# shgaurav1/DVG

Measured on AMD Instinct MI355X. Metric: predicted frames/sec at 64x64, batch 64, 10-in/10-out, higher is better.
Workload: dtype f32; 1 GPU; Moving-MNIST 64x64 rollout (generate_frames.py make_gifs sample loop), vgg_64 + lstm + GP trigger sample at i%15==0, batch 64 per GPU, 10-in/10-out; model_family=vgg, batch_per_gpu=64, n_past=10, n_future=10, parallelism=replicas x1 (no data-path collective), launch=hipGraph replay, rollouts_in_flight=3, tile_policy=energy, loop_invariant_skip_halves=hoisted, upsample_conv3x3=as transposed 4x4/s2 conv, conv3x3_deep_layers=Winograd F(4x4,3x3) / F(2x2,3x3)

## Files before the change

dvg_amd/csrc/conv_igemm2.hip:

```cpp
#include <cstdlib>
#include <type_traits>

#include "dvg_common.h"

namespace dvg {

constexpr int DVG_GEMM_WGS_PER_CU = DVG_BF16X3 ? 3 : 4;
constexpr int DVG_GEMM128_WGS = DVG_BF16X3 ? 3 : 2;
constexpr int DVG_GEMM128_GT = DVG_BF16X3 ? 2 : 4;
constexpr int DVG_GEMM_GT = 4;
constexpr int DVG_GEMM128_MIN_WGS = 4 * 768;
[[maybe_unused]] constexpr int DVG_GEMM_NT2 = 256;
constexpr int DVG_TILE16_MIN_WGS = 256;

enum { M2_CONV3 = 0, M2_CONV4S2 = 1, M2_CONVT4S2 = 2, M2_GEMM = 3 };

struct Igemm2Params {
    const float* x;
    const float* skip;
    const float* w;
    const float* scale;
    const float* shift;
    float* y;
    float* y_pool;
// ... 1273 lines not shown
    const long total = (long)cout * cin * 12 / 2;
    const int nblk = cout >> 6;
    for (long i = blockIdx.x * (long)blockDim.x + threadIdx.x; i < total; i += (long)gridDim.x * blockDim.x) {
        const int k = (int)(i & 7) * 2;
        long r = i >> 3;
        const int co = r % cout; r /= cout;
        const int tap = r % 12;
        const int chunk = r / 12;
        const int row = tap >> 2, f = tap & 3;
        float u[2];
#pragma unroll
        for (int e = 0; e < 2; ++e) {
            const float* g = src + (((long)co * cin + chunk * 16 + k + e) * 3 + row) * 3;
            if (f == 0) u[e] = g[0];
            else if (f == 1) u[e] = ((g[0] + g[1]) + g[2]) * 0.5f;
            else if (f == 2) u[e] = ((g[0] - g[1]) + g[2]) * 0.5f;
            else u[e] = g[2];
        }
        wrow_store_pair(dst, (((size_t)chunk * nblk + (co >> 6)) * 12 + tap) * 64 + (co & 63), co & 63, k, u[0], u[1]);
    }
    wrow_drain();
}

__global__ void pack_k16_kernel(const float* __restrict__ src, float* __restrict__ dst, int cout, int cin, int kh,
                                int kw, int transposed) {
    const long total = (long)cout * cin * kh * kw / 2;
    const int nblk = cout >> 6, taps = kh * kw;
    for (long i = blockIdx.x * (long)blockDim.x + threadIdx.x; i < total; i += (long)gridDim.x * blockDim.x) {
        const int k = (int)(i & 7) * 2;
        long r = i >> 3;
        const int co = r % cout; r /= cout;
        const int t = r % taps;
        const int chunk = r / taps;
        const int ci = chunk * 16 + k, a = t / kw, b = t % kw;
        const long j = transposed ? ((((long)ci * cout + co) * kh + (kh - 1 - a)) * kw + (kw - 1 - b))
                                  : ((((long)co * cin + ci) * kh + a) * kw + b);
        const long j1 = j + (transposed ? (long)cout * kh * kw : (long)kh * kw);
        int slot = t;
        if (transposed && kh == 4 && kw == 4) {
            const int py = a & 1, px = b & 1;
            slot = (py * 2 + px) * 4 + ((2 + py - a) >> 1) * 2 + ((2 + px - b) >> 1);
        } else if (kh == 4 && kw == 4) {
            slot = ((a & 1) * 2 + (b & 1)) * 4 + (a >> 1) * 2 + (b >> 1);
        }
        wrow_store_pair(dst, (((size_t)chunk * nblk + (co >> 6)) * taps + slot) * 64 + (co & 63), co & 63, k, src[j], src[j1]);
    }
    wrow_drain();
}

}

using namespace dvg;

extern "C" int dvg_mfma_mode(void) { return DVG_BF16X3 ? 1 : 0; }
extern "C" int dvg_packed_row_floats(void) { return DVG_WROW; }

extern "C" void dvg_debug_set_clockbuf(void* buf, unsigned records) {
    g_clk = (unsigned long long*)buf;
    g_clk_cap = buf ? records : 0;
}

extern "C" int dvg_pack_conv_weight_k16(const float* w, float* w_packed, int cout, int cin, int kh, int kw,
                                        int transposed, void* stream) {
    DVG_REQUIRE(w && w_packed, DVG_ERR_NULL, "dvg_pack_conv_weight_k16: NULL pointer");
    DVG_REQUIRE(cout > 0 && cout % 64 == 0 && cin > 0 && cin % 16 == 0 && kh > 0 && kw > 0, DVG_ERR_SHAPE,
                "dvg_pack_conv_weight_k16: Cin must be a multiple of 16, Cout of 64");
    const long total = (long)cout * cin * kh * kw / 2;
    long g = (total + 255) / 256;
    if (g > 4096) g = 4096;
    hipLaunchKernelGGL(pack_k16_kernel, dim3((unsigned)g), dim3(256), 0, (hipStream_t)stream, w, w_packed, cout, cin, kh,
                       kw, transposed);
    return check_launch("dvg_pack_conv_weight_k16");
}

static long v2_wgs(int mode, int N, int Hg, int Wg, int Cout, int ti, int th, int tw) {
    return (long)((N + ti - 1) / ti) * (Hg / th) * (Wg / tw) * (Cout / 64) * (mode == M2_CONVT4S2 ? 4 : 1);
}

static int v2_splits(int mode, int N, int Hg, int Wg, int Cout, int Cin, int ti, int th, int tw) {
    if (tw == 16) return 1;
    return choose_splitk(v2_wgs(mode, N, Hg, Wg, Cout, ti, th, tw), Cin / 16);
}

extern "C" int dvg_conv_splitk_v2(int mode, int N, int H, int W, int Cin, int Cout) {
    int Hg = H, Wg = W;
    if (mode == M2_CONV4S2) { Hg = H / 2; Wg = W / 2; }
    int ti, th, tw;
    if (Cin % 16 || Cout % 64 || tile2(mode, N, Hg, Wg, Cout, &ti, &th, &tw)) return -1;
    return v2_splits(mode, N, Hg, Wg, Cout, Cin, ti, th, tw);
}

extern "C" int dvg_conv_stats_rows_v2(int mode, int N, int H, int W, int Cin, int Cout, int pool, int with_workspace) {
    int Hg = H, Wg = W;
    if (mode == M2_CONV4S2) { Hg = H / 2; Wg = W / 2; }
    int ti, th, tw;
    if (tile2(mode, N, Hg, Wg, Cout, &ti, &th, &tw)) return -1;
    if (with_workspace && v2_splits(mode, N, Hg, Wg, Cout, Cin, ti, th, tw) > 1) {
        int Ho = H, Wo = W;
        if (mode == M2_CONV4S2) { Ho = H / 2; Wo = W / 2; }
        if (mode == M2_CONVT4S2) { Ho = 2 * H; Wo = 2 * W; }
        const long units = pool ? (long)N * (Ho / 2) * (Wo / 2) : (long)N * Ho * Wo;
        const int upb = finish_units_per_block(units);
        return (int)((units + upb - 1) / upb);
    }
    return ((N + ti - 1) / ti) * (Hg / th) * (Wg / tw) * (mode == M2_CONVT4S2 ? 4 : 1);
}

static int checks2(const Igemm2Params& p, const char* who) {
    DVG_REQUIRE(p.x && p.w && p.y, DVG_ERR_NULL, "%s: x/w/y must not be NULL", who);
    DVG_REQUIRE((p.skip != nullptr) == (p.C2 > 0), DVG_ERR_SHAPE, "%s: skip pointer / C2 mismatch", who);
    DVG_REQUIRE(p.N > 0 && p.H > 0 && p.W > 0, DVG_ERR_SHAPE, "%s: empty shape", who);
    DVG_REQUIRE(p.C1 > 0 && p.C1 % 16 == 0 && p.C2 % 16 == 0, DVG_ERR_SHAPE, "%s: C1=%d C2=%d must be multiples of 16",
                who, p.C1, p.C2);
    DVG_REQUIRE(p.Cout > 0 && p.Cout % 64 == 0, DVG_ERR_SHAPE, "%s: Cout=%d must be a multiple of 64", who, p.Cout);
    DVG_REQUIRE(aligned16(p.x) && aligned16(p.w) && aligned16(p.y) && aligned16(p.skip), DVG_ERR_ALIGN,
                "%s: pointers must be 16-byte aligned", who);
    DVG_REQUIRE(p.act >= DVG_ACT_NONE && p.act <= DVG_ACT_SIGMOID, DVG_ERR_SHAPE, "%s: bad act", who);
    return DVG_OK;
}

#define D2(MODE, TI_, TH_, TW_) \
    if (ti == TI_ && th == TH_ && tw == TW_)                                             \
        return launch2<MODE, TI_, TH_, TW_>(p, Hg, Wg, workspace, workspace_floats, (hipStream_t)stream);



extern "C" int dvg_conv3x3_bn_act_v2(const float* x, const float* skip, const float* w_k16, const float* scale,
                                     const float* shift, float* y, float* y_pool, float* stats, int N, int H, int W,
                                     int C1, int C2, int Cout, int upsample_x, int act, float slope,
                                     float* workspace, long workspace_floats, const float* addend,
                                     const int* addend_map, int addend_block, void* stream) {
    Igemm2Params p{x, skip, w_k16, scale, shift, y, y_pool, stats, N, H, W, C1, C2, Cout, upsample_x ? 1 : 0, act, slope,
                   0, 0, 0, 0, 0, 1, 0, nullptr};
    p.addend = addend;
    p.add_map = addend ? addend_map : nullptr;
    p.add_B = addend_block;
    DVG_REQUIRE(p.add_map == nullptr || (addend_block > 0 && N % addend_block == 0), DVG_ERR_SHAPE,
                "dvg_conv3x3_bn_act_v2: addend_block must divide N");
    if (int e = checks2(p, "dvg_conv3x3_bn_act_v2")) return e;
    DVG_REQUIRE(aligned16(addend) && (addend == nullptr || y_pool == nullptr), DVG_ERR_SHAPE,
                "dvg_conv3x3_bn_act_v2: addend must be 16-byte aligned and excludes the pooled output");
    DVG_REQUIRE(H % 8 == 0 && W % 8 == 0, DVG_ERR_SHAPE, "dvg_conv3x3_bn_act_v2: H=%d W=%d must be multiples of 8", H, W);
    int Hg = H, Wg = W, ti, th, tw;
    DVG_REQUIRE(tile2(M2_CONV3, N, Hg, Wg, Cout, &ti, &th, &tw) == 0 && ti == 1, DVG_ERR_SHAPE,
                "dvg_conv3x3_bn_act_v2: no tile for %dx%d", H, W);
    D2(M2_CONV3, 1, 8, 16)
    D2(M2_CONV3, 1, 8, 8)
    return fail(DVG_ERR_SHAPE, "dvg_conv3x3_bn_act_v2: no kernel");
}

extern "C" int dvg_conv3x3_first_pair(const float* frame, const float* w0, const float* scale0, const float* shift0,
                                      const float* w1_k16, const float* scale1, const float* shift1, float* y, float* y_pool,
                                      int N, int H, int W, int Cout, int act, float slope, int y_from, void* stream) {
    DVG_REQUIRE(frame && w0 && scale0 && shift0, DVG_ERR_NULL, "dvg_conv3x3_first_pair: NULL pointer");
    DVG_REQUIRE(y_from >= 0 && y_from <= N && (y_from == 0 || y_pool != nullptr) && (y != nullptr || y_from == N), DVG_ERR_SHAPE,
                "dvg_conv3x3_first_pair: y_from=%d needs 0 <= y_from <= N, a pooled output when > 0, y unless == N", y_from);
    float* const y_biased = y ? y - (size_t)y_from * H * W * Cout : y_pool;
    Igemm2Params p{frame , nullptr, w1_k16, scale1, shift1, y_biased, y_pool, nullptr, N, H, W, 64, 0, Cout, 0,
                   act, slope, 0, 0, 0, 0, 0, 1, 0, nullptr};
    p.first_frame = frame; p.first_w = w0; p.first_scale = scale0; p.first_shift = shift0; p.first_slope = 0.2f;
    p.y_from = y_from;
    if (int e = checks2(p, "dvg_conv3x3_first_pair")) return e;
    DVG_REQUIRE(H % 8 == 0 && W % 16 == 0 && (long)N * (H / 8) * (W / 16) * (Cout / 64) >= 512, DVG_ERR_SHAPE,
                "dvg_conv3x3_first_pair: H %% 8, W %% 16 and >= 512 workgroups needed (N=%d H=%d W=%d Cout=%d)", N, H, W, Cout);
    return launch2<M2_CONV3, 1, 8, 16, 1, true>(p, H, W, nullptr, 0, (hipStream_t)stream);
}

extern "C" int dvg_pack_conv_weight_wx(const float* w, float* w_packed, int cout, int cin, void* stream) {
    DVG_REQUIRE(w && w_packed, DVG_ERR_NULL, "dvg_pack_conv_weight_wx: NULL pointer");
    DVG_REQUIRE(cout > 0 && cout % 64 == 0 && cin > 0 && cin % 16 == 0, DVG_ERR_SHAPE,
                "dvg_pack_conv_weight_wx: Cin must be a multiple of 16, Cout of 64");
    DVG_REQUIRE(aligned16(w_packed), DVG_ERR_ALIGN, "dvg_pack_conv_weight_wx: w_packed must be 16-byte aligned");
    const long total = (long)cout * cin * 12 / 2;
    hipLaunchKernelGGL(pack_wx_kernel, dim3(grid_for(total, 256, 4096)), dim3(256), 0, (hipStream_t)stream, w, w_packed, cout, cin);
    return check_launch("dvg_pack_conv_weight_wx");
}

static int checks_wx(const Igemm2Params& p, const char* who) {
    DVG_REQUIRE(p.N > 0 && p.H > 0 && p.W > 0, DVG_ERR_SHAPE, "%s: empty shape", who);
    DVG_REQUIRE(p.C1 > 0 && p.C1 % 16 == 0 && p.C2 == 0 && p.skip == nullptr && !p.upsample, DVG_ERR_SHAPE,
                "%s: Cin=%d must be a multiple of 16; no concat operand, no upsampling", who, p.C1 + p.C2);
    DVG_REQUIRE(p.Cout > 0 && p.Cout % 64 == 0, DVG_ERR_SHAPE, "%s: Cout=%d must be a multiple of 64", who, p.Cout);
    DVG_REQUIRE(p.H % 8 == 0 && p.W % 16 == 0, DVG_ERR_SHAPE, "%s: H=%d must be a multiple of 8, W=%d of 16", who, p.H, p.W);
    DVG_REQUIRE((long)p.H * p.W * p.Cout < (1L << 31), DVG_ERR_SHAPE, "%s: image of %d x %d x %d floats too large", who, p.H, p.W, p.Cout);
    DVG_REQUIRE(aligned16(p.x) && aligned16(p.w) && aligned16(p.y) && aligned16(p.y_pool) && aligned16(p.addend), DVG_ERR_ALIGN,
                "%s: pointers must be 16-byte aligned", who);
    DVG_REQUIRE(p.act >= DVG_ACT_NONE && p.act <= DVG_ACT_SIGMOID, DVG_ERR_SHAPE, "%s: bad act", who);
    DVG_REQUIRE(DVG_BF16X3 != 0, DVG_ERR_SHAPE, "%s: the f32-MFMA build has no WX kernel", who);
    return DVG_OK;
}

extern "C" int dvg_conv3x3_bn_act_wx(const float* x, const float* skip, const float* w_wx, const float* scale,
                                     const float* shift, float* y, float* y_pool, int N, int H, int W, int C1, int C2,
                                     int Cout, int upsample_x, int act, float slope, const float* addend,
                                     const int* addend_map, int addend_block, void* stream) {
    const char* who = "dvg_conv3x3_bn_act_wx";
    DVG_REQUIRE(x && w_wx && y, DVG_ERR_NULL, "%s: x/w/y must not be NULL", who);
    Igemm2Params p{x, skip, w_wx, scale, shift, y, y_pool, nullptr, N, H, W, C1, C2, Cout, upsample_x ? 1 : 0, act, slope,
                   0, 0, 0, 0, 0, 1, 0, nullptr};
    p.addend = addend;
    p.add_map = addend ? addend_map : nullptr;
    p.add_B = addend_block;
    DVG_REQUIRE(p.add_map == nullptr || (addend_block > 0 && N % addend_block == 0), DVG_ERR_SHAPE, "%s: addend_block must divide N", who);
    DVG_REQUIRE(addend == nullptr || y_pool == nullptr, DVG_ERR_SHAPE, "%s: addend excludes the pooled output", who);
    if (int e = checks_wx(p, who)) return e;
#if DVG_BF16X3
    return launch_wx<false>(p, (hipStream_t)stream);
#else
    return DVG_ERR_SHAPE;
#endif
}

extern "C" int dvg_conv3x3_first_pair_wx(const float* frame, const float* w0, const float* scale0, const float* shift0,
                                         const float* w1_wx, const float* scale1, const float* shift1, float* y, float* y_pool,
                                         int N, int H, int W, int Cout, int act, float slope, int y_from, void* stream) {
    const char* who = "dvg_conv3x3_first_pair_wx";
    DVG_REQUIRE(frame && w0 && scale0 && shift0 && w1_wx, DVG_ERR_NULL, "%s: NULL pointer", who);
    DVG_REQUIRE(y_from >= 0 && y_from <= N && (y_from == 0 || y_pool != nullptr) && (y != nullptr || y_from == N), DVG_ERR_SHAPE,
                "%s: y_from=%d needs 0 <= y_from <= N, a pooled output when > 0, y unless == N", who, y_from);
    DVG_REQUIRE(aligned16(w0) && aligned16(scale0) && aligned16(shift0) && aligned16(y), DVG_ERR_ALIGN,
                "%s: pointers must be 16-byte aligned", who);
    float* const y_biased = y ? y - (size_t)y_from * H * W * Cout : y_pool;
    Igemm2Params p{frame , nullptr, w1_wx, scale1, shift1, y_biased, y_pool, nullptr, N, H, W, 64, 0, Cout, 0,
                   act, slope, 0, 0, 0, 0, 0, 1, 0, nullptr};
    p.first_frame = frame; p.first_w = w0; p.first_scale = scale0; p.first_shift = shift0; p.first_slope = 0.2f;
    p.y_from = y_from;
    if (int e = checks_wx(p, who)) return e;
#if DVG_BF16X3
    return launch_wx<true>(p, (hipStream_t)stream);
#else
    return DVG_ERR_SHAPE;
#endif
}

extern "C" int dvg_conv4x4s2_bn_act_v2(const float* x, const float* w_k16, const float* scale, const float* shift,
                                       float* y, float* stats, int N, int H, int W, int Cin, int Cout, int act,
                                       float slope, float* workspace, long workspace_floats, void* stream) {
    Igemm2Params p{x, nullptr, w_k16, scale, shift, y, nullptr, stats, N, H, W, Cin, 0, Cout, 0, act, slope, 0, 0, 0, 0, 0,
                   1, 0, nullptr};
    if (int e = checks2(p, "dvg_conv4x4s2_bn_act_v2")) return e;
    DVG_REQUIRE(H % 2 == 0 && W % 2 == 0, DVG_ERR_SHAPE, "dvg_conv4x4s2_bn_act_v2: odd input");
    DVG_REQUIRE((long)N * H * W * Cin < (1L << 31), DVG_ERR_SHAPE,
                "dvg_conv4x4s2_bn_act_v2: input of %d x %d x %d x %d floats too large (32-bit offsets)", N, H, W, Cin);
    int Hg = H / 2, Wg = W / 2, ti, th, tw;
    DVG_REQUIRE(tile2(M2_CONV4S2, N, Hg, Wg, Cout, &ti, &th, &tw) == 0, DVG_ERR_SHAPE,
                "dvg_conv4x4s2_bn_act_v2: unsupported map %dx%d", H, W);
    D2(M2_CONV4S2, 1, 8, 16)
    D2(M2_CONV4S2, 1, 8, 8)
    D2(M2_CONV4S2, 4, 4, 4)
    return fail(DVG_ERR_SHAPE, "dvg_conv4x4s2_bn_act_v2: no kernel");
}

extern "C" int dvg_convT4x4s2_bn_act_v2(const float* x, const float* skip, const float* w_k16, const float* scale,
                                        const float* shift, float* y, float* stats, int N, int H, int W, int C1,
                                        int C2, int Cout, int act, float slope, float* workspace, long workspace_floats,
                                        const float* addend, const int* addend_map, int addend_block, void* stream) {
    Igemm2Params p{x, skip, w_k16, scale, shift, y, nullptr, stats, N, H, W, C1, C2, Cout, 0, act, slope, 0, 0, 0, 0, 0,
                   1, 0, nullptr};
    p.addend = addend;
    p.add_map = addend ? addend_map : nullptr;
    p.add_B = addend_block;
    DVG_REQUIRE(p.add_map == nullptr || (addend_block > 0 && N % addend_block == 0), DVG_ERR_SHAPE,
                "dvg_convT4x4s2_bn_act_v2: addend_block must divide N");
    if (int e = checks2(p, "dvg_convT4x4s2_bn_act_v2")) return e;
    DVG_REQUIRE(aligned16(addend), DVG_ERR_ALIGN, "dvg_convT4x4s2_bn_act_v2: addend must be 16-byte aligned");
    int Hg = H, Wg = W, ti, th, tw;
    DVG_REQUIRE(tile2(M2_CONVT4S2, N, Hg, Wg, Cout, &ti, &th, &tw) == 0, DVG_ERR_SHAPE,
                "dvg_convT4x4s2_bn_act_v2: unsupported map %dx%d", H, W);
    D2(M2_CONVT4S2, 1, 8, 16)
    D2(M2_CONVT4S2, 1, 8, 8)
    D2(M2_CONVT4S2, 4, 4, 4)
    return fail(DVG_ERR_SHAPE, "dvg_convT4x4s2_bn_act_v2: no kernel");
}

extern "C" int dvg_convT4x4s2_bn_act_proj(const float* x, const float* w_k16, const float* scale, const float* shift,
                                          const float* proj_w, float* proj_out, int T, int N, int H, int W, int C1, int Cout,
                                          int act, float slope, const float* addend, const int* addend_map, int addend_block,
                                          void* stream) {
    const char* who = "dvg_convT4x4s2_bn_act_proj";
    DVG_REQUIRE(x && w_k16 && proj_w && proj_out, DVG_ERR_NULL, "%s: x / w / proj_w / proj_out must not be NULL", who);
    DVG_REQUIRE(N > 0 && H > 0 && W > 0, DVG_ERR_SHAPE, "%s: empty shape", who);
    DVG_REQUIRE(C1 > 0 && C1 % 16 == 0, DVG_ERR_SHAPE, "%s: C1=%d must be a multiple of 16", who, C1);
    DVG_REQUIRE(Cout == 64, DVG_ERR_SHAPE, "%s: Cout=%d must be 64 (one column block holds every channel of a pixel)", who, Cout);
    DVG_REQUIRE(T >= 1 && T <= 48, DVG_ERR_SHAPE, "%s: T=%d must be in 1..48", who, T);
    DVG_REQUIRE(aligned16(x) && aligned16(w_k16) && aligned16(proj_w) && aligned16(addend), DVG_ERR_ALIGN,
                "%s: pointers must be 16-byte aligned", who);
    DVG_REQUIRE(act >= DVG_ACT_NONE && act <= DVG_ACT_SIGMOID, DVG_ERR_SHAPE, "%s: bad act", who);
    Igemm2Params p{x, nullptr, w_k16, scale, shift, nullptr, nullptr, nullptr, N, H, W, C1, 0, Cout, 0, act, slope, 0, 0, 0, 0, 0,
                   1, 0, nullptr};
    p.addend = addend;
    p.add_map = addend ? addend_map : nullptr;
    p.add_B = addend_block;
    DVG_REQUIRE(p.add_map == nullptr || (addend_block > 0 && N % addend_block == 0), DVG_ERR_SHAPE, "%s: addend_block must divide N", who);
    p.proj_w = proj_w;
    p.proj_out = proj_out;
    p.proj_T = T;
    int ti, th, tw;
    DVG_REQUIRE(tile2(M2_CONVT4S2, N, H, W, Cout, &ti, &th, &tw) == 0 && ti == 1, DVG_ERR_SHAPE,
                "%s: unsupported map %dx%d (multiples of 8 needed)", who, H, W);
    if (tw == 16) return launch2<M2_CONVT4S2, 1, 8, 16, 1, false, true>(p, H, W, nullptr, 0, (hipStream_t)stream);
    return launch2<M2_CONVT4S2, 1, 8, 8, 1, false, true>(p, H, W, nullptr, 0, (hipStream_t)stream);
}

extern "C" int dvg_gemm_batched_k16(const float* x, const float* w_k16, float* y, int NB, int H, int W, int Cin, int Cout,
                                    void* stream) {
    Igemm2Params p{x, nullptr, w_k16, nullptr, nullptr, y, nullptr, nullptr, NB, H, W, Cin, 0, Cout, 0, DVG_ACT_NONE, 0.f,
                   0, 0, 0, 0, 0, 1, 0, nullptr};
    if (int e = checks2(p, "dvg_gemm_batched_k16")) return e;
    DVG_REQUIRE(Cin % (16 * DVG_GEMM_GT) == 0 && H % 8 == 0 && W % 8 == 0, DVG_ERR_SHAPE,
                "dvg_gemm_batched_k16: Cin=%d must be a multiple of %d, H=%d W=%d multiples of 8", Cin, 16 * DVG_GEMM_GT, H, W);
    DVG_REQUIRE((long)H * W * Cin < (1L << 31), DVG_ERR_SHAPE, "dvg_gemm_batched_k16: image of %d x %d x %d floats too large", H, W, Cin);
    p.w_image_stride = (long)Cin / 16 * Cout * DVG_WROW;
    float* workspace = nullptr;
    const long workspace_floats = 0;
    const int Hg = H, Wg = W, ti = 1, th = 8;
    int tw, nt;
    DVG_REQUIRE(gemm_tile(NB, Hg, Wg, Cout, &tw, &nt) == 0, DVG_ERR_SHAPE, "dvg_gemm_batched_k16: no tile for %dx%d", H, W);
#if DVG_BF16X3
    if (nt == 2) return launch2<M2_GEMM, 1, 8, 16, 2>(p, Hg, Wg, workspace, workspace_floats, (hipStream_t)stream);
#endif
    D2(M2_GEMM, 1, 8, 16)
    D2(M2_GEMM, 1, 8, 8)
    return fail(DVG_ERR_SHAPE, "dvg_gemm_batched_k16: no kernel");
}

extern "C" int dvg_gemm_batched_plan(int NB, int H, int W, int Cin, int Cout, int* tile_w, int* nt, int* ni) {
    if (!tile_w || !nt || !ni || NB <= 0 || H <= 0 || W <= 0 || Cin <= 0 || Cout <= 0) return -1;
    if (Cin % (16 * DVG_GEMM_GT) || Cout % 64 || H % 8 || W % 8) return -1;
    if (gemm_tile(NB, H, W, Cout, tile_w, nt)) return -1;
    *ni = gemm_images_per_wg(*tile_w, *nt, NB, H, W, Cout);
    return 0;
}
```

dvg_amd/csrc/winograd.hip:

```cpp
#include <cstdlib>

#include "dvg_common.h"

namespace dvg {

__global__ void winograd_weight_kernel(const float* __restrict__ w, float* __restrict__ u, int cout, int cin) {
    const unsigned total = (unsigned)cout * (unsigned)cin / 2;
    for (unsigned i = blockIdx.x * blockDim.x + threadIdx.x; i < total; i += gridDim.x * blockDim.x) {
        const unsigned rr = i >> 3;
        const int co = (int)(rr % (unsigned)cout), chunk = (int)(rr / (unsigned)cout), k = (int)(i & 7) * 2;
        const float* g = w + ((size_t)co * cin + chunk * 16 + k) * 9;
        float t[2][4][3];
#pragma unroll
        for (int e = 0; e < 2; ++e)
#pragma unroll
            for (int s = 0; s < 3; ++s) {
                const float g0 = g[9 * e + s], g1 = g[9 * e + 3 + s], g2 = g[9 * e + 6 + s];
                t[e][0][s] = g0;
                t[e][1][s] = 0.5f * (g0 + g1 + g2);
                t[e][2][s] = 0.5f * (g0 - g1 + g2);
                t[e][3][s] = g2;
            }
        const unsigned row0 = ((unsigned)(co >> 6) * (unsigned)(cin / 16) + (unsigned)chunk) * 64u + (unsigned)(co & 63);
        const unsigned pos_rows = (unsigned)(cout >> 6) * (unsigned)(cin / 16) * 64u;
#pragma unroll
        for (int a = 0; a < 4; ++a) {
            float r[2][4];
#pragma unroll
            for (int e = 0; e < 2; ++e) {
                r[e][0] = t[e][a][0];
                r[e][1] = 0.5f * (t[e][a][0] + t[e][a][1] + t[e][a][2]);
                r[e][2] = 0.5f * (t[e][a][0] - t[e][a][1] + t[e][a][2]);
                r[e][3] = t[e][a][2];
            }
#pragma unroll
            for (int b = 0; b < 4; ++b)
                wrow_store_pair(u, (size_t)(a * 4 + b) * pos_rows + row0, co & 63, k, r[0][b], r[1][b]);
        }
    }
    wrow_drain();
}

__global__ __launch_bounds__(256) void winograd_input_kernel(const float* __restrict__ x, float* __restrict__ v, int N,
                                                             int H, int W, int C4) {
    const int Ht = H >> 1, Wt = W >> 1;
    const long T = (long)N * Ht * Wt, total = T * C4;
    for (long i = blockIdx.x * (long)blockDim.x + threadIdx.x; i < total; i += (long)gridDim.x * blockDim.x) {
        const int c4 = (int)(i % C4);
        const long t = i / C4;
        const int tx = (int)(t % Wt);
        const long r = t / Wt;
        const int ty = (int)(r % Ht), n = (int)(r / Ht);
        f32x4 d[4][4];
#pragma unroll
        for (int a = 0; a < 4; ++a) {
            const int yy = 2 * ty - 1 + a;
#pragma unroll
            for (int b = 0; b < 4; ++b) {
                const int xx = 2 * tx - 1 + b;
                const bool ok = (unsigned)yy < (unsigned)H && (unsigned)xx < (unsigned)W;
                d[a][b] = ok ? reinterpret_cast<const f32x4*>(x)[(((size_t)n * H + yy) * W + xx) * C4 + c4]
                             : f32x4{0.f, 0.f, 0.f, 0.f};
            }
        }
        f32x4 e[4][4];
#pragma unroll
        for (int b = 0; b < 4; ++b) {
            e[0][b] = d[0][b] - d[2][b];
            e[1][b] = d[1][b] + d[2][b];
            e[2][b] = d[2][b] - d[1][b];
            e[3][b] = d[1][b] - d[3][b];
        }
#pragma unroll
        for (int a = 0; a < 4; ++a) {
            const f32x4 o0 = e[a][0] - e[a][2], o1 = e[a][1] + e[a][2], o2 = e[a][2] - e[a][1], o3 = e[a][1] - e[a][3];
            f32x4* dst = reinterpret_cast<f32x4*>(v) + ((size_t)(a * 4) * T + t) * C4 + c4;
            dst[0] = o0;
            dst[(size_t)T * C4] = o1;
            dst[(size_t)2 * T * C4] = o2;
            dst[(size_t)3 * T * C4] = o3;
        }
    }
}

template <bool POOL>
__global__ __launch_bounds__(256) void winograd_output_kernel(const float* __restrict__ m, const float* __restrict__ scale,
                                                              const float* __restrict__ shift, float* __restrict__ y,
                                                              float* __restrict__ y_pool, int N, int H, int W, int C4,
                                                              int act, float slope, int y_from) {
    const int Ht = H >> 1, Wt = W >> 1;
    const long T = (long)N * Ht * Wt, total = T * C4;
    for (long i = blockIdx.x * (long)blockDim.x + threadIdx.x; i < total; i += (long)gridDim.x * blockDim.x) {
        const int c4 = (int)(i % C4);
        const long t = i / C4;
        const int tx = (int)(t % Wt);
        const long r = t / Wt;
        const int ty = (int)(r % Ht), n = (int)(r / Ht);
        f32x4 q[4][4];
#pragma unroll
        for (int a = 0; a < 4; ++a)
#pragma unroll
            for (int b = 0; b < 4; ++b) q[a][b] = reinterpret_cast<const f32x4*>(m)[((size_t)(a * 4 + b) * T + t) * C4 + c4];
        f32x4 s0[4], s1[4];
#pragma unroll
        for (int b = 0; b < 4; ++b) {
            s0[b] = q[0][b] + q[1][b] + q[2][b];
            s1[b] = q[1][b] - q[2][b] - q[3][b];
        }
        f32x4 o[2][2];
        o[0][0] = s0[0] + s0[1] + s0[2];
        o[0][1] = s0[1] - s0[2] - s0[3];
        o[1][0] = s1[0] + s1[1] + s1[2];
        o[1][1] = s1[1] - s1[2] - s1[3];
        const f32x4 sc = scale ? reinterpret_cast<const f32x4*>(scale)[c4] : f32x4{1.f, 1.f, 1.f, 1.f};
        const f32x4 sf = shift ? reinterpret_cast<const f32x4*>(shift)[c4] : f32x4{0.f, 0.f, 0.f, 0.f};
        f32x4 mx;
#pragma unroll
        for (int pp = 0; pp < 2; ++pp)
#pragma unroll
            for (int qq = 0; qq < 2; ++qq) {
                f32x4 val;
#pragma unroll
                for (int k = 0; k < 4; ++k) val[k] = apply_act(o[pp][qq][k] * sc[k] + sf[k], act, slope);
                if (!POOL || n >= y_from)
                    reinterpret_cast<f32x4*>(y)[(((size_t)(n - y_from) * H + 2 * ty + pp) * W + 2 * tx + qq) * C4 + c4] = val;
                if (POOL) {
                    if (pp == 0 && qq == 0) mx = val;
                    else
#pragma unroll
                        for (int k = 0; k < 4; ++k) mx[k] = fmaxf(mx[k], val[k]);
                }
            }
        if (POOL) reinterpret_cast<f32x4*>(y_pool)[(((size_t)n * Ht + ty) * Wt + tx) * C4 + c4] = mx;
    }
}

typedef float f32x2 __attribute__((ext_vector_type(2)));
template <typename V> struct VecN { static constexpr int N = sizeof(V) / 4; };
template <typename V> __device__ __forceinline__ float vget(const V& v, int k) { return v[k]; }
template <> __device__ __forceinline__ float vget<float>(const float& v, int) { return v; }
template <typename V> __device__ __forceinline__ void vset(V& v, int k, float x) { v[k] = x; }
template <> __device__ __forceinline__ void vset<float>(float& v, int, float x) { v = x; }
template <typename V> __device__ __forceinline__ V vzero() { V z; for (int k = 0; k < VecN<V>::N; ++k) vset(z, k, 0.f); return z; }

template <typename V>
__device__ __forceinline__ void bt4(const V (&d)[6], V (&e)[6]) {
    e[0] = 4.f * d[0] - 5.f * d[2] + d[4];
    e[1] = -4.f * (d[1] + d[2]) + d[3] + d[4];
    e[2] = 4.f * (d[1] - d[2]) - d[3] + d[4];
    e[3] = 2.f * (d[3] - d[1]) - d[2] + d[4];
    e[4] = 2.f * (d[1] - d[3]) - d[2] + d[4];
    e[5] = 4.f * d[1] - 5.f * d[3] + d[5];
}

template <typename V>
__device__ __forceinline__ void at4(const V (&q)[6], V (&o)[4]) {
    const V a = q[1] + q[2], b = q[1] - q[2], c = q[3] + q[4], d = q[3] - q[4];
    o[0] = q[0] + a + c;
    o[1] = b + 2.f * d;
    o[2] = a + 4.f * c;
    o[3] = b + 8.f * d + q[5];
}

__global__ void winograd4_weight_kernel(const float* __restrict__ w, float* __restrict__ u, int cout, int cin) {
    const float G[6][3] = {{0.25f, 0.f, 0.f}, {-1.f / 6, -1.f / 6, -1.f / 6}, {-1.f / 6, 1.f / 6, -1.f / 6},
                           {1.f / 24, 1.f / 12, 1.f / 6}, {1.f / 24, -1.f / 12, 1.f / 6}, {0.f, 0.f, 1.f}};
    const unsigned total = (unsigned)cout * (unsigned)cin / 2;
    for (unsigned i = blockIdx.x * blockDim.x + threadIdx.x; i < total; i += gridDim.x * blockDim.x) {
        const unsigned r = i >> 3;
        const int co = (int)(r % (unsigned)cout), chunk = (int)(r / (unsigned)cout), k = (int)(i & 7) * 2;
        const float* g = w + ((size_t)co * cin + chunk * 16 + k) * 9;
        float t[2][6][3];
#pragma unroll
        for (int e = 0; e < 2; ++e)
#pragma unroll
            for (int a = 0; a < 6; ++a)
#pragma unroll
                for (int s2 = 0; s2 < 3; ++s2)
                    t[e][a][s2] = G[a][0] * g[9 * e + s2] + G[a][1] * g[9 * e + 3 + s2] + G[a][2] * g[9 * e + 6 + s2];
        const unsigned row0 = ((unsigned)(co >> 6) * (unsigned)(cin / 16) + (unsigned)chunk) * 64u + (unsigned)(co & 63);
        const unsigned pos_rows = (unsigned)(cout >> 6) * (unsigned)(cin / 16) * 64u;
#pragma unroll
        for (int a = 0; a < 6; ++a)
#pragma unroll
            for (int b = 0; b < 6; ++b)
                wrow_store_pair(u, (size_t)(a * 6 + b) * pos_rows + row0, co & 63, k,
                                t[0][a][0] * G[b][0] + t[0][a][1] * G[b][1] + t[0][a][2] * G[b][2],
                                t[1][a][0] * G[b][0] + t[1][a][1] * G[b][1] + t[1][a][2] * G[b][2]);
    }
    wrow_drain();
}

template <typename V>
__global__ __launch_bounds__(256) void winograd4_input_kernel(const float* __restrict__ x, float* __restrict__ v, int N,
                                                              int H, int W, int C4, long Tt, long t_off, int up) {
    const int Ht = H >> 2, Wt = W >> 2, Hs = H >> up, Ws = W >> up;
    const long T = (long)N * Ht * Wt, total = T * C4;
    for (long i = blockIdx.x * (long)blockDim.x + threadIdx.x; i < total; i += (long)gridDim.x * blockDim.x) {
        const int c4 = (int)(i % C4);
        const long t = i / C4;
        const int tx = (int)(t % Wt);
        const long r = t / Wt;
        const int ty = (int)(r % Ht), n = (int)(r / Ht);
        V e[6][6];
#pragma unroll
        for (int b = 0; b < 6; ++b) {
            const int xx = 4 * tx - 1 + b;
            V d[6];
#pragma unroll
            for (int a = 0; a < 6; ++a) {
                const int yy = 4 * ty - 1 + a;
                const bool ok = (unsigned)yy < (unsigned)H && (unsigned)xx < (unsigned)W;
                d[a] = ok ? reinterpret_cast<const V*>(x)[(((size_t)n * Hs + (yy >> up)) * Ws + (xx >> up)) * C4 + c4] : vzero<V>();
            }
            V col[6];
            bt4(d, col);
#pragma unroll
            for (int a = 0; a < 6; ++a) e[a][b] = col[a];
        }
#pragma unroll
        for (int a = 0; a < 6; ++a) {
            V o[6];
            bt4(e[a], o);
#pragma unroll
            for (int b = 0; b < 6; ++b) reinterpret_cast<V*>(v)[((size_t)(a * 6 + b) * Tt + t_off + t) * C4 + c4] = o[b];
        }
    }
}

template <typename V>
__device__ __forceinline__ void a4(const V (&d)[4], V (&o)[6]) {
    const V s02 = d[0] + d[2], s13 = d[1] + d[3], t = d[0] + 4.f * d[2], u = 2.f * d[1] + 8.f * d[3];
    o[0] = d[0];
    o[1] = s02 + s13;
    o[2] = s02 - s13;
    o[3] = t + u;
    o[4] = t - u;
    o[5] = d[3];
}

template <typename V>
__global__ __launch_bounds__(256) void winograd4_dy_kernel(const float* __restrict__ dy, float* __restrict__ dm, int N, int H,
                                                           int W, int C4, long Tt, long t_off) {
    const int Ht = H >> 2, Wt = W >> 2;
    const long T = (long)N * Ht * Wt, total = T * C4;
    for (long i = blockIdx.x * (long)blockDim.x + threadIdx.x; i < total; i += (long)gridDim.x * blockDim.x) {
        const int c4 = (int)(i % C4);
        const long t = i / C4;
        const int tx = (int)(t % Wt);
        const long r = t / Wt;
        const int ty = (int)(r % Ht), n = (int)(r / Ht);
        V e[6][4];
#pragma unroll
        for (int b = 0; b < 4; ++b) {
            V d[4];
#pragma unroll
            for (int a = 0; a < 4; ++a)
                d[a] = reinterpret_cast<const V*>(dy)[(((size_t)n * H + 4 * ty + a) * W + 4 * tx + b) * C4 + c4];
            V col[6];
            a4(d, col);
#pragma unroll
            for (int a = 0; a < 6; ++a) e[a][b] = col[a];
        }
#pragma unroll
        for (int a = 0; a < 6; ++a) {
            V o[6];
            a4(e[a], o);
#pragma unroll
            for (int b = 0; b < 6; ++b) reinterpret_cast<V*>(dm)[((size_t)(a * 6 + b) * Tt + t_off + t) * C4 + c4] = o[b];
        }
    }
}

template <bool POOL, typename V>

__global__ __launch_bounds__(256) void winograd4_output_kernel(const float* __restrict__ m, const float* __restrict__ scale,
                                                               const float* __restrict__ shift, float* __restrict__ y,
                                                               float* __restrict__ y_pool, int N, int H, int W, int C4,
                                                               int act, float slope, const float* __restrict__ addend,
                                                               int y_from) {
    constexpr int VN = VecN<V>::N;
    const int Ht = H >> 2, Wt = W >> 2;
    const long T = (long)N * Ht * Wt, total = T * C4;
    for (long i = blockIdx.x * (long)blockDim.x + threadIdx.x; i < total; i += (long)gridDim.x * blockDim.x) {
        const int c4 = (int)(i % C4);
        const long t = i / C4;
        const int tx = (int)(t % Wt);
        const long r = t / Wt;
        const int ty = (int)(r % Ht), n = (int)(r / Ht);
        V s[4][6];
#pragma unroll
        for (int b = 0; b < 6; ++b) {
            V q[6];
#pragma unroll
            for (int a = 0; a < 6; ++a) q[a] = reinterpret_cast<const V*>(m)[((size_t)(a * 6 + b) * T + t) * C4 + c4];
            V col[4];
            at4(q, col);
#pragma unroll
            for (int pp = 0; pp < 4; ++pp) s[pp][b] = col[pp];
        }
        V sc, sf;
#pragma unroll
        for (int k = 0; k < VN; ++k) {
            vset(sc, k, scale ? scale[c4 * VN + k] : 1.f);
            vset(sf, k, shift ? shift[c4 * VN + k] : 0.f);
        }
        V val[4][4];
#pragma unroll
        for (int pp = 0; pp < 4; ++pp) {
            V o[4];
            at4(s[pp], o);
#pragma unroll
            for (int qq = 0; qq < 4; ++qq) {
                const size_t px = (((size_t)n * H + 4 * ty + pp) * W + 4 * tx + qq) * C4 + c4;
                V ad = vzero<V>();
                if (addend) ad = reinterpret_cast<const V*>(addend)[px];
#pragma unroll
                for (int k = 0; k < VN; ++k)
                    vset(val[pp][qq], k, apply_act((vget(o[qq], k) + vget(ad, k)) * vget(sc, k) + vget(sf, k), act, slope));
                if (!POOL || n >= y_from) reinterpret_cast<V*>(y)[px - (size_t)y_from * H * W * C4] = val[pp][qq];
            }
        }
        if (POOL) {
#pragma unroll
            for (int pp = 0; pp < 2; ++pp)
#pragma unroll
                for (int qq = 0; qq < 2; ++qq) {
                    V mx;
#pragma unroll
                    for (int k = 0; k < VN; ++k)
                        vset(mx, k, fmaxf(fmaxf(vget(val[2 * pp][2 * qq], k), vget(val[2 * pp][2 * qq + 1], k)),
                                          fmaxf(vget(val[2 * pp + 1][2 * qq], k), vget(val[2 * pp + 1][2 * qq + 1], k))));
                    reinterpret_cast<V*>(y_pool)[(((size_t)n * (H >> 1) + 2 * ty + pp) * (W >> 1) + 2 * tx + qq) * C4 + c4] = mx;
                }
        }
    }
}

template <int HW>
__global__ __launch_bounds__(256) void winograd4_out_in_kernel(const float* __restrict__ m, const float* __restrict__ scale,
                                                               const float* __restrict__ shift, float* __restrict__ v, int N,
                                                               int C, int act, float slope, const float* __restrict__ addend) {
    constexpr int WT = HW / 4, TI = WT * WT, CS = 256 / TI;
    __shared__ float ys[HW * HW * CS];
    const int tid = threadIdx.x, cl = tid % CS, t_img = tid / CS, ty = t_img / WT, tx = t_img % WT;
    const int cblocks = C / CS;
    const int n = blockIdx.x / cblocks, c = (blockIdx.x % cblocks) * CS + cl;
    const long T = (long)N * TI, t = (long)n * TI + t_img;
    {
        float sq[4][6];
#pragma unroll
        for (int b = 0; b < 6; ++b) {
            float q[6];
#pragma unroll
            for (int a = 0; a < 6; ++a) q[a] = m[((size_t)(a * 6 + b) * T + t) * C + c];
            float col[4];
            at4(q, col);
#pragma unroll
            for (int pp = 0; pp < 4; ++pp) sq[pp][b] = col[pp];
        }
        const float sc = scale ? scale[c] : 1.f, sf = shift ? shift[c] : 0.f;
#pragma unroll
        for (int pp = 0; pp < 4; ++pp) {
            float o[4];
            at4(sq[pp], o);
#pragma unroll
            for (int qq = 0; qq < 4; ++qq) {
                const float ad = addend ? addend[(((size_t)n * HW + 4 * ty + pp) * HW + 4 * tx + qq) * C + c] : 0.f;
                ys[((4 * ty + pp) * HW + 4 * tx + qq) * CS + cl] = apply_act((o[qq] + ad) * sc + sf, act, slope);
            }
        }
    }
    __syncthreads();
    float e[6][6];
#pragma unroll
    for (int b = 0; b < 6; ++b) {
        const int xx = 4 * tx - 1 + b;
        float d[6];
#pragma unroll
        for (int a = 0; a < 6; ++a) {
            const int yy = 4 * ty - 1 + a;
            d[a] = ((unsigned)yy < (unsigned)HW && (unsigned)xx < (unsigned)HW) ? ys[(yy * HW + xx) * CS + cl] : 0.f;
        }
        float col[6];
        bt4(d, col);
#pragma unroll
        for (int a = 0; a < 6; ++a) e[a][b] = col[a];
    }
#pragma unroll
    for (int a = 0; a < 6; ++a) {
        float o[6];
        bt4(e[a], o);
#pragma unroll
        for (int b = 0; b < 6; ++b) v[((size_t)(a * 6 + b) * T + t) * C + c] = o[b];
    }
}

template <int HW, int CS, typename V, bool POOL, int NT, bool UP = false>
__global__ __launch_bounds__(NT) void winograd4_chain_kernel(const float* __restrict__ m, const float* __restrict__ scale,
                                                             const float* __restrict__ shift, float* __restrict__ y,
                                                             float* __restrict__ v, int N, int C, int act, float slope,
                                                             const float* __restrict__ addend, int y_from) {
    constexpr int VN = VecN<V>::N;
    constexpr int WT = HW / 4, TI = WT * WT;
    static_assert(!(POOL && UP), "pool and upsample exclude each other");
    constexpr int SS = POOL ? HW / 2 : HW;
    constexpr int S2 = UP ? 2 * HW : SS;
    constexpr int WT2 = S2 / 4, TI2 = WT2 * WT2;
    constexpr int CV = CS / VN;
    extern __shared__ __attribute__((aligned(16))) float chain_ys[];
    float* const ys = chain_ys;
    const int cblocks = C / CS;
    const int n = blockIdx.x / cblocks, c0 = (blockIdx.x % cblocks) * CS;
    const int CVg = C / VN;
    const long T = (long)N * TI;
    for (int u = threadIdx.x; u < TI * CV; u += NT) {
        const int cv = u % CV, t_img = u / CV, ty = t_img / WT, tx = t_img % WT;
        const long t = (long)n * TI + t_img;
        const int cg = c0 / VN + cv;
        V s[4][6];
#pragma unroll
        for (int b = 0; b < 6; ++b) {
            V q[6];
#pragma unroll
            for (int a = 0; a < 6; ++a) q[a] = __builtin_nontemporal_load(reinterpret_cast<const V*>(m) + ((size_t)(a * 6 + b) * T + t) * CVg + cg);
            V col[4];
            at4(q, col);
#pragma unroll
            for (int pp = 0; pp < 4; ++pp) s[pp][b] = col[pp];
        }
        V sc, sf;
#pragma unroll
        for (int k = 0; k < VN; ++k) {
            vset(sc, k, scale ? scale[c0 + cv * VN + k] : 1.f);
            vset(sf, k, shift ? shift[c0 + cv * VN + k] : 0.f);
        }
        V val[4][4];
#pragma unroll
        for (int pp = 0; pp < 4; ++pp) {
            V o[4];
            at4(s[pp], o);
#pragma unroll
            for (int qq = 0; qq < 4; ++qq) {
                V ad = vzero<V>();
                if (addend) ad = reinterpret_cast<const V*>(addend)[(((size_t)n * HW + 4 * ty + pp) * HW + 4 * tx + qq) * CVg + cg];
#pragma unroll
                for (int k = 0; k < VN; ++k)
                    vset(val[pp][qq], k, apply_act((vget(o[qq], k) + vget(ad, k)) * vget(sc, k) + vget(sf, k), act, slope));
                if (POOL) {
                    if (n >= y_from)
                        reinterpret_cast<V*>(y)[(((size_t)(n - y_from) * HW + 4 * ty + pp) * HW + 4 * tx + qq) * CVg + cg] = val[pp][qq];
                } else
                    *reinterpret_cast<V*>(&ys[((4 * ty + pp) * HW + 4 * tx + qq) * CS + cv * VN]) = val[pp][qq];
            }
        }
        if (POOL) {
#pragma unroll
            for (int pp = 0; pp < 2; ++pp)
#pragma unroll
                for (int qq = 0; qq < 2; ++qq) {
                    V mx;
#pragma unroll
                    for (int k = 0; k < VN; ++k)
                        vset(mx, k, fmaxf(fmaxf(vget(val[2 * pp][2 * qq], k), vget(val[2 * pp][2 * qq + 1], k)),
                                          fmaxf(vget(val[2 * pp + 1][2 * qq], k), vget(val[2 * pp + 1][2 * qq + 1], k))));
                    *reinterpret_cast<V*>(&ys[((2 * ty + pp) * SS + 2 * tx + qq) * CS + cv * VN]) = mx;
                }
        }
    }
    __syncthreads();
    const long T2 = (long)N * TI2;
    for (int u = threadIdx.x; u < TI2 * CV; u += NT) {
        const int cv = u % CV, t_img = u / CV, ty = t_img / WT2, tx = t_img % WT2;
        const long t2 = (long)n * TI2 + t_img;
        const int cg = c0 / VN + cv;
        V e[6][6];
#pragma unroll
        for (int b = 0; b < 6; ++b) {
            const int xx = 4 * tx - 1 + b;
            V d[6];
#pragma unroll
            for (int a = 0; a < 6; ++a) {
                const int yy = 4 * ty - 1 + a;
                d[a] = ((unsigned)yy < (unsigned)S2 && (unsigned)xx < (unsigned)S2)
                           ? *reinterpret_cast<const V*>(&ys[((yy >> (UP ? 1 : 0)) * SS + (xx >> (UP ? 1 : 0))) * CS + cv * VN])
                           : vzero<V>();
            }
            V col[6];
            bt4(d, col);
#pragma unroll
            for (int a = 0; a < 6; ++a) e[a][b] = col[a];
        }
#pragma unroll
        for (int a = 0; a < 6; ++a) {
            V o[6];
            bt4(e[a], o);
#pragma unroll
            for (int b = 0; b < 6; ++b) reinterpret_cast<V*>(v)[((size_t)(a * 6 + b) * T2 + t2) * CVg + cg] = o[b];
        }
    }
}

template <int HW, int CS, typename V, bool POOL, int NT, bool UP = false>
static int launch_chain(const float* mm, const float* scale, const float* shift, float* y, float* v, int N, int C, int act,
                        float slope, hipStream_t st, const float* addend = nullptr, int y_from = 0) {
    constexpr int S2 = POOL ? HW / 2 : HW;
    constexpr size_t lds = (size_t)S2 * S2 * CS * 4;
    auto kern = winograd4_chain_kernel<HW, CS, V, POOL, NT, UP>;
    static bool attr = false;
    if (!attr && lds > 48 * 1024) {
        hipError_t e = hipFuncSetAttribute(reinterpret_cast<const void*>(kern), hipFuncAttributeMaxDynamicSharedMemorySize, (int)lds);
        if (e != hipSuccess) return fail(DVG_ERR_HIP, "hipFuncSetAttribute: %s", hipGetErrorString(e));
        attr = true;
    }
    hipLaunchKernelGGL(kern, dim3((unsigned)((long)N * (C / CS))), dim3(NT), lds, st, mm, scale, shift, y, v, N, C, act, slope,
                       addend, y_from);
    return check_launch("winograd4_chain");
}

template <int KP>
__global__ __launch_bounds__(256) void stem_up_input_kernel(const float* __restrict__ vec, int ldv, const float* __restrict__ wt,
                                                            const float* __restrict__ scale, const float* __restrict__ shift,
                                                            float* __restrict__ v, int M, int C, int K, int act, float slope) {
    constexpr int BR = 8;
    __shared__ float vs[BR * KP];
    __shared__ float ys[BR * 16 * 16];
    const int tid = threadIdx.x, cl = tid & 15, hw = tid >> 4;
    const int c = blockIdx.x * 16 + cl;
    const size_t N = (size_t)16 * C, n = (size_t)hw * C + c;
    const int m0 = blockIdx.y * BR, mrows = min(BR, M - m0);
    for (int i = tid; i < BR * KP; i += 256) {
        const int r = i / KP, k = i % KP;
        vs[i] = (r < mrows && k < K) ? vec[(size_t)(m0 + r) * ldv + k] : 0.f;
    }
    float w[KP];
#pragma unroll
    for (int k = 0; k < KP; ++k) w[k] = wt[(size_t)k * N + n];
    __syncthreads();
    const float sc = scale ? scale[c] : 1.f, sf = shift ? shift[c] : 0.f;
#pragma unroll
    for (int bb = 0; bb < BR; ++bb) {
        const f32x4* vr = reinterpret_cast<const f32x4*>(vs + bb * KP);
        float s0 = 0.f, s1 = 0.f;
#pragma unroll
        for (int k4 = 0; k4 < KP / 4; ++k4) {
            const f32x4 v4 = vr[k4];
            s0 = fmaf(v4[0], w[4 * k4], s0);
            s1 = fmaf(v4[1], w[4 * k4 + 1], s1);
            s0 = fmaf(v4[2], w[4 * k4 + 2], s0);
            s1 = fmaf(v4[3], w[4 * k4 + 3], s1);
        }
        ys[(bb * 16 + hw) * 16 + cl] = apply_act((s0 + s1) * sc + sf, act, slope);
    }
    __syncthreads();
    const long T = (long)M * 4;
    for (int u = tid; u < BR * 64; u += 256) {
        const int ucl = u & 15, tile = (u >> 4) & 3, bb = u >> 6;
        if (bb >= mrows) continue;
        const int ty = tile >> 1, tx = tile & 1;
        const float* src = ys + bb * 256 + ucl;
        float e[6][6];
#pragma unroll
        for (int b = 0; b < 6; ++b) {
            const int xx = 4 * tx - 1 + b;
            float d[6];
#pragma unroll
            for (int a = 0; a < 6; ++a) {
                const int yy = 4 * ty - 1 + a;
                d[a] = ((unsigned)yy < 8u && (unsigned)xx < 8u) ? src[((yy >> 1) * 4 + (xx >> 1)) * 16] : 0.f;
            }
            float col[6];
            bt4(d, col);
#pragma unroll
            for (int a = 0; a < 6; ++a) e[a][b] = col[a];
        }
        const long t = (long)(m0 + bb) * 4 + tile;
        float* dst = v + t * C + blockIdx.x * 16 + ucl;
#pragma unroll
        for (int a = 0; a < 6; ++a) {
            float o[6];
            bt4(e[a], o);
#pragma unroll
            for (int b = 0; b < 6; ++b) dst[(size_t)(a * 6 + b) * T * C] = o[b];
        }
    }
}

static int wino4_width(long tiles, int C) {
    if (tiles * (C / 4) >= 1024L * 256) return 4;
    if (tiles * (C / 2) >= 1024L * 256) return 2;
    return 1;
}

static int chain_variant() { return 0; }

static inline unsigned wgrid(long n) {
    long g = (n + 255) / 256;
    return (unsigned)(g > 16384 ? 16384 : (g < 1 ? 1 : g));
}

}

using namespace dvg;

extern "C" int dvg_winograd_weight(const float* w_oihw, float* u_k16, int cout, int cin, int m, void* stream) {
    DVG_REQUIRE(w_oihw && u_k16, DVG_ERR_NULL, "dvg_winograd_weight: NULL pointer");
    DVG_REQUIRE(cout > 0 && cout % 64 == 0 && cin > 0 && cin % 16 == 0 && (m == 2 || m == 4), DVG_ERR_SHAPE,
                "dvg_winograd_weight: Cin must be a multiple of 16, Cout of 64, m 2 or 4");
    if (m == 2)
        hipLaunchKernelGGL(winograd_weight_kernel, dim3(wgrid((long)cout * cin / 2)), dim3(256), 0, (hipStream_t)stream, w_oihw,
                           u_k16, cout, cin);
    else
        hipLaunchKernelGGL(winograd4_weight_kernel, dim3(wgrid((long)cout * cin / 2)), dim3(256), 0, (hipStream_t)stream, w_oihw,
                           u_k16, cout, cin);
    return check_launch("dvg_winograd_weight");
}

extern "C" int dvg_winograd_input(const float* x, float* v, int N, int H, int W, int C, int m, int upsample, void* stream) {
    DVG_REQUIRE(x && v, DVG_ERR_NULL, "dvg_winograd_input: NULL pointer");
    DVG_REQUIRE((m == 2 || m == 4) && N > 0 && H > 0 && W > 0 && H % m == 0 && W % m == 0 && C > 0 && C % 4 == 0,
                DVG_ERR_SHAPE, "dvg_winograd_input: m 2 or 4, H and W multiples of m, C %% 4 == 0 needed");
    DVG_REQUIRE(upsample == 0 || (upsample == 1 && m == 4 && H % 2 == 0 && W % 2 == 0), DVG_ERR_SHAPE,
                "dvg_winograd_input: upsample needs m = 4 and even H, W");
    const int up = upsample;
    DVG_REQUIRE(aligned16(x) && aligned16(v), DVG_ERR_ALIGN, "dvg_winograd_input: alignment");
    const long tiles = (long)N * (H / m) * (W / m);
    const hipStream_t st = (hipStream_t)stream;
    if (m == 2) {
        hipLaunchKernelGGL(winograd_input_kernel, dim3(wgrid(tiles * (C / 4))), dim3(256), 0, st, x, v, N, H, W, C / 4);
    } else {
        const int cw = wino4_width(tiles, C);
        if (cw == 4)
            hipLaunchKernelGGL(winograd4_input_kernel<f32x4>, dim3(wgrid(tiles * (C / 4))), dim3(256), 0, st, x, v, N, H, W, C / 4, tiles, 0L, up);
        else if (cw == 2)
            hipLaunchKernelGGL(winograd4_input_kernel<f32x2>, dim3(wgrid(tiles * (C / 2))), dim3(256), 0, st, x, v, N, H, W, C / 2, tiles, 0L, up);
        else
            hipLaunchKernelGGL(winograd4_input_kernel<float>, dim3(wgrid(tiles * C)), dim3(256), 0, st, x, v, N, H, W, C, tiles, 0L, up);
    }
    return check_launch("dvg_winograd_input");
}

extern "C" int dvg_winograd_transform_width(long tiles, int C) {
    if (tiles <= 0 || C <= 0 || C % 4) return 0;
    return wino4_width(tiles, C);
}

extern "C" int dvg_winograd_wgrad_operands(const float* x, const float* dy, float* v, float* dm, int N, int H, int W, int Cin,
                                           int Cout, long t_total, long t_off, void* stream) {
    DVG_REQUIRE((x && v) || (dy && dm), DVG_ERR_NULL, "dvg_winograd_wgrad_operands: nothing to do");
    DVG_REQUIRE(N > 0 && H > 0 && W > 0 && H % 4 == 0 && W % 4 == 0 && Cin > 0 && Cin % 4 == 0 && Cout > 0 && Cout % 4 == 0,
                DVG_ERR_SHAPE, "dvg_winograd_wgrad_operands: H and W multiples of 4, channels multiples of 4 needed");
    const long tiles = (long)N * (H / 4) * (W / 4);
    DVG_REQUIRE(t_off >= 0 && t_off + tiles <= t_total, DVG_ERR_SHAPE,
                "dvg_winograd_wgrad_operands: tiles [%ld, %ld) outside the buffer of %ld", t_off, t_off + tiles, t_total);
    DVG_REQUIRE(aligned16(x) && aligned16(dy) && aligned16(v) && aligned16(dm), DVG_ERR_ALIGN,
                "dvg_winograd_wgrad_operands: alignment");
    const hipStream_t st = (hipStream_t)stream;
#define WOPS(KERNEL_, SRC_, DST_, C_, ...)                                                                                        \
    do {                                                                                                                       \
        const int cw_ = wino4_width(tiles, (C_));                                                                              \
        if (cw_ == 4)                                                                                                          \
            hipLaunchKernelGGL(KERNEL_<f32x4>, dim3(wgrid(tiles * ((C_) / 4))), dim3(256), 0, st, SRC_, DST_, N, H, W, (C_) / 4, t_total, t_off __VA_ARGS__); \
        else if (cw_ == 2)                                                                                                     \
            hipLaunchKernelGGL(KERNEL_<f32x2>, dim3(wgrid(tiles * ((C_) / 2))), dim3(256), 0, st, SRC_, DST_, N, H, W, (C_) / 2, t_total, t_off __VA_ARGS__); \
        else                                                                                                                   \
            hipLaunchKernelGGL(KERNEL_<float>, dim3(wgrid(tiles * (C_))), dim3(256), 0, st, SRC_, DST_, N, H, W, (C_), t_total, t_off __VA_ARGS__);           \
    } while (0)
    if (x && v) {
        WOPS(winograd4_input_kernel, x, v, Cin, , 0);
        if (int e = check_launch("dvg_winograd_wgrad_operands (input)")) return e;
    }
    if (dy && dm) {
        WOPS(winograd4_dy_kernel, dy, dm, Cout, );
        if (int e = check_launch("dvg_winograd_wgrad_operands (dy)")) return e;
    }
#undef WOPS
    return DVG_OK;
}

extern "C" int dvg_winograd_output_input(const float* mm, const float* scale, const float* shift, float* v_next, int N, int H,
                                         int W, int C, int act, float slope, const float* addend, void* stream) {
    DVG_REQUIRE(mm && v_next, DVG_ERR_NULL, "dvg_winograd_output_input: NULL pointer");
    DVG_REQUIRE(aligned16(addend), DVG_ERR_ALIGN, "dvg_winograd_output_input: addend alignment");
    DVG_REQUIRE(N > 0 && H == W && (H == 8 || H == 16 || H == 32) && C > 0 && C % 64 == 0, DVG_ERR_SHAPE,
                "dvg_winograd_output_input: 8x8, 16x16 or 32x32 maps, C %% 64 == 0 needed (got %dx%d, C=%d)", H, W, C);
    DVG_REQUIRE(act >= 0 && act <= 3, DVG_ERR_SHAPE, "dvg_winograd_output_input: bad act");
    DVG_REQUIRE(aligned16(mm) && aligned16(v_next), DVG_ERR_ALIGN, "dvg_winograd_output_input: alignment");
    const hipStream_t st = (hipStream_t)stream;
    const int var = chain_variant();
    if (H == 8) {
        hipLaunchKernelGGL(winograd4_out_in_kernel<8>, dim3((unsigned)((long)N * (C / 64))), dim3(256), 0, st, mm, scale, shift,
                           v_next, N, C, act, slope, addend);
    } else if (H == 16) {
        if (var == 9) {
            hipLaunchKernelGGL(winograd4_out_in_kernel<16>, dim3((unsigned)((long)N * (C / 16))), dim3(256), 0, st, mm, scale,
                               shift, v_next, N, C, act, slope, addend);
        } else if (var == 2 || (var == 0 && (long)N * (C / 64) < 1024)) {
            return launch_chain<16, 32, float, false, 512>(mm, scale, shift, nullptr, v_next, N, C, act, slope, st, addend);
        } else {
            return launch_chain<16, 64, f32x2, false, 512>(mm, scale, shift, nullptr, v_next, N, C, act, slope, st, addend);
        }
    } else {
        if (var == 1) return launch_chain<32, 16, f32x2, false, 512>(mm, scale, shift, nullptr, v_next, N, C, act, slope, st, addend);
        return launch_chain<32, 32, f32x4, false, 512>(mm, scale, shift, nullptr, v_next, N, C, act, slope, st, addend);
    }
    return check_launch("dvg_winograd_output_input");
}

extern "C" int dvg_stem_up_winograd_input(const float* vec, int ldv, const float* w_kn, int KP, const float* scale,
                                          const float* shift, float* v_next, int M, int C, int K, int act, float slope,
                                          void* stream) {
    DVG_REQUIRE(vec && w_kn && v_next, DVG_ERR_NULL, "dvg_stem_up_winograd_input: NULL pointer");
    DVG_REQUIRE(M > 0 && C > 0 && C % 16 == 0 && K > 0 && K <= KP && (KP == 96 || KP == 128) && ldv >= K, DVG_ERR_SHAPE,
                "dvg_stem_up_winograd_input: bad shape M=%d C=%d K=%d KP=%d (C %% 16 == 0, KP 96 or 128)", M, C, K, KP);
    DVG_REQUIRE(act >= 0 && act <= 3, DVG_ERR_SHAPE, "dvg_stem_up_winograd_input: bad act");
    DVG_REQUIRE(aligned16(v_next), DVG_ERR_ALIGN, "dvg_stem_up_winograd_input: alignment");
    const dim3 grid(C / 16, (M + 7) / 8);
    if (KP == 96)
        hipLaunchKernelGGL(stem_up_input_kernel<96>, grid, dim3(256), 0, (hipStream_t)stream, vec, ldv, w_kn, scale, shift, v_next,
                           M, C, K, act, slope);
    else
        hipLaunchKernelGGL(stem_up_input_kernel<128>, grid, dim3(256), 0, (hipStream_t)stream, vec, ldv, w_kn, scale, shift, v_next,
                           M, C, K, act, slope);
    return check_launch("dvg_stem_up_winograd_input");
}

extern "C" int dvg_winograd_output_up_input(const float* mm, const float* scale, const float* shift, float* v_next, int N, int H,
                                            int W, int C, int act, float slope, void* stream) {
    DVG_REQUIRE(mm && v_next, DVG_ERR_NULL, "dvg_winograd_output_up_input: NULL pointer");
    DVG_REQUIRE(N > 0 && H == W && H == 8 && C > 0 && C % 64 == 0, DVG_ERR_SHAPE,
                "dvg_winograd_output_up_input: 8x8 maps, C %% 64 == 0 needed (got %dx%d, C=%d)", H, W, C);
    DVG_REQUIRE(act >= 0 && act <= 3, DVG_ERR_SHAPE, "dvg_winograd_output_up_input: bad act");
    DVG_REQUIRE(aligned16(mm) && aligned16(v_next), DVG_ERR_ALIGN, "dvg_winograd_output_up_input: alignment");
    const hipStream_t st = (hipStream_t)stream;
    return launch_chain<8, 32, float, false, 512, true>(mm, scale, shift, nullptr, v_next, N, C, act, slope, st);
}

extern "C" int dvg_winograd_output_pool_input(const float* mm, const float* scale, const float* shift, float* y, float* v_next,
                                              int N, int H, int W, int C, int act, float slope, int y_from, void* stream) {
    DVG_REQUIRE(mm && v_next && (y || y_from == N), DVG_ERR_NULL, "dvg_winograd_output_pool_input: NULL pointer");
    DVG_REQUIRE(y_from >= 0 && y_from <= N, DVG_ERR_SHAPE, "dvg_winograd_output_pool_input: y_from=%d outside [0, N]", y_from);
    DVG_REQUIRE(N > 0 && H == W && (H == 16 || H == 32) && C > 0 && C % 64 == 0, DVG_ERR_SHAPE,
                "dvg_winograd_output_pool_input: 16x16 or 32x32 maps, C %% 64 == 0 needed (got %dx%d, C=%d)", H, W, C);
    DVG_REQUIRE(act >= 0 && act <= 3, DVG_ERR_SHAPE, "dvg_winograd_output_pool_input: bad act");
    DVG_REQUIRE(aligned16(mm) && aligned16(y) && aligned16(v_next), DVG_ERR_ALIGN, "dvg_winograd_output_pool_input: alignment");
    const hipStream_t st = (hipStream_t)stream;
    const int var = chain_variant();
    (void)var;
    if (H == 16) return launch_chain<16, 64, f32x2, true, 512>(mm, scale, shift, y, v_next, N, C, act, slope, st, nullptr, y_from);
    return launch_chain<32, 32, f32x2, true, 1024>(mm, scale, shift, y, v_next, N, C, act, slope, st, nullptr, y_from);
}

extern "C" int dvg_winograd_output(const float* m, const float* scale, const float* shift, float* y, float* y_pool, int N,
                                   int H, int W, int C, int act, float slope, int mt, const float* addend, int y_from,
                                   void* stream) {
    DVG_REQUIRE(m && (y || (y_pool && y_from == N)), DVG_ERR_NULL, "dvg_winograd_output: NULL pointer");
    DVG_REQUIRE(y_from >= 0 && y_from <= N && (y_from == 0 || y_pool != nullptr), DVG_ERR_SHAPE,
                "dvg_winograd_output: y_from=%d needs 0 <= y_from <= N and a pooled output", y_from);
    DVG_REQUIRE(addend == nullptr || (mt == 4 && y_pool == nullptr && aligned16(addend)), DVG_ERR_SHAPE,
                "dvg_winograd_output: addend needs m = 4, no pooled output, 16-byte alignment");
    DVG_REQUIRE((mt == 2 || mt == 4) && N > 0 && H > 0 && W > 0 && H % mt == 0 && W % mt == 0 && C > 0 && C % 4 == 0,
                DVG_ERR_SHAPE, "dvg_winograd_output: m 2 or 4, H and W multiples of m, C %% 4 == 0 needed");
    DVG_REQUIRE(act >= 0 && act <= 3, DVG_ERR_SHAPE, "dvg_winograd_output: bad act");
    DVG_REQUIRE(aligned16(m) && aligned16(y) && aligned16(y_pool) && aligned16(scale) && aligned16(shift), DVG_ERR_ALIGN,
                "dvg_winograd_output: alignment");
    const unsigned g = wgrid((long)N * (H / mt) * (W / mt) * (C / 4));
    const hipStream_t st = (hipStream_t)stream;
    if (mt == 2 && y_pool)
        hipLaunchKernelGGL(winograd_output_kernel<true>, dim3(g), dim3(256), 0, st, m, scale, shift, y, y_pool, N, H, W, C / 4, act, slope, y_from);
    else if (mt == 2)
        hipLaunchKernelGGL(winograd_output_kernel<false>, dim3(g), dim3(256), 0, st, m, scale, shift, y, y_pool, N, H, W, C / 4, act, slope, 0);
    else {
        const long tiles = (long)N * (H / 4) * (W / 4);
#define W4OUT(POOL_, V_, CW_)                                                                                             \
    hipLaunchKernelGGL((winograd4_output_kernel<POOL_, V_>), dim3(wgrid(tiles * (C / CW_))), dim3(256), 0, st, m, scale, shift, \
                       y, y_pool, N, H, W, C / CW_, act, slope, addend, y_from)
        const int cw = wino4_width(tiles, C);
        if (cw == 4) { if (y_pool) W4OUT(true, f32x4, 4); else W4OUT(false, f32x4, 4); }
        else if (cw == 2) { if (y_pool) W4OUT(true, f32x2, 2); else W4OUT(false, f32x2, 2); }
        else { if (y_pool) W4OUT(true, float, 1); else W4OUT(false, float, 1); }
#undef W4OUT
    }
    return check_launch("dvg_winograd_output");
}
```

dvg_amd/fused.py:

```python
from __future__ import annotations

import collections
import contextlib
import functools
import os
import types
import weakref

import torch
import torch.nn as nn

from . import _derived, ops, weights
from ._derived import derived, version_key as _ver
from .ops import ACT_LRELU, ACT_NONE, ACT_SIGMOID, ACT_TANH, MODE_CONV3, MODE_CONV4S2, MODE_CONVT4S2


WINOGRAD = int(os.environ.get("DVG_WINOGRAD", "4"))
if WINOGRAD not in (0, 2, 4):
    raise RuntimeError("DVG_WINOGRAD must be 0, 2 or 4")


_WINO_MIN_C = 64
_WINO_MAX_HW = 32


WINOGRAD_LAYER_OVERRIDE = {}


def winograd_tile(n, c, h, w, cout) -> int:
    if WINOGRAD_LAYER_OVERRIDE:
        forced = WINOGRAD_LAYER_OVERRIDE.get((c, h, cout))
        if forced is not None:
            return forced if (forced == 0 or ops.winograd_ok(n, c, h, w, cout, forced)) else 0
    if WINOGRAD >= 4 and c >= _WINO_MIN_C and h <= _WINO_MAX_HW and w <= _WINO_MAX_HW and ops.winograd_ok(n, c, h, w, cout, 4):
        return 4
    if WINOGRAD >= 2 and c >= 256 and ops.winograd_ok(n, c, h, w, cout, 2) and \
            ((h <= 8 and w <= 8) or (h <= 16 and w <= 16 and cout >= 256)):
        return 2
    return 0


UPCONV_WINOGRAD = True
_UPCONV_WINO_MAX = 16


def folded_affine(conv: nn.Module, bn: nn.BatchNorm2d):
    def build():
        with torch.no_grad():
            inv = torch.rsqrt(bn.running_var + bn.eps)
            scale = (bn.weight * inv) if bn.weight is not None else inv
            bias = conv.bias if conv.bias is not None else torch.zeros_like(bn.running_mean)
            shift = (bias - bn.running_mean) * scale
            if bn.bias is not None:
                shift = shift + bn.bias
            return scale.contiguous(), shift.contiguous()

    return derived(bn, "fold", (conv.bias, bn.weight, bn.bias, bn.running_mean, bn.running_var), build)


def _needs_grad(*ts) -> bool:
    return torch.is_grad_enabled() and any(
        t is not None and (t.t if isinstance(t, ops.SharedBlocks) else t).requires_grad for t in ts)


def _no_shared(skip, who):
    if isinstance(skip, ops.SharedBlocks):
        raise RuntimeError(f"{who}: shared skip blocks (time-batched decoder calls) are a training-path operand (autograd)")


def _bias(conv):
    return conv.bias.detach() if conv.bias is not None else None


Block = collections.namedtuple("Block", "raw mode finish cat dgrad")


def _raw_conv3(x, skip, wp, b, *, up=False, stats=False, addend=None):
    return ops.conv3x3(x, skip, wp, None, b, upsample=up, act=ACT_NONE, stats=stats, addend=addend)


def _raw_convT4s2(x, skip, wp, b, *, up=False, stats=False, addend=None):
    if up:
        raise RuntimeError("convT4s2: no fused upsampling")
    return ops.convT4x4s2(x, skip, wp, None, b, act=ACT_NONE, stats=stats, addend=addend)


def _raw_plain(name):
    def raw(x, skip, w, b, *, up=False, stats=False, addend=None):
        if skip is not None or up or addend is not None:
            raise RuntimeError(f"{name}: neither a concat conv nor an upsampling one")
        return getattr(ops, name)(x, w, None, b, act=ACT_NONE, stats=stats)
    return raw


def _dgrad_conv3(du, weight, lo, hi):
    n, c, h, w = du.shape
    m = winograd_tile(n, c, h, w, hi - lo)
    if m:
        return ops.conv3x3_winograd(du, weights.winograd(weight, m, lo, hi, dgrad=True), None, None, act=ACT_NONE)
    return ops.conv3x3(du, None, weights.packed(weight, True, lo, hi, 1), None, None, act=ACT_NONE)


def _dgrad_conv4s2(du, weight, lo, hi):
    return ops.convT4x4s2(du, None, weights.packed(weight, True, lo, hi, 1), None, None, act=ACT_NONE)


def _dgrad_convT4s2(du, weight, lo, hi):
    return ops.conv4x4s2(du, weights.packed(weight, False, lo, hi, 0), None, None, act=ACT_NONE)


BLOCKS = {
    "conv3": Block(_raw_conv3, MODE_CONV3, (0, 3, 3), 1, _dgrad_conv3),
    "conv4s2": Block(_raw_plain("conv4x4s2"), MODE_CONV4S2, (0, 4, 4), 1, _dgrad_conv4s2),
    "convT4s2": Block(_raw_convT4s2, MODE_CONVT4S2, (1, 4, 4), 0, _dgrad_convT4s2),
    "conv3_first": Block(_raw_plain("conv3x3_first"), None, (0, 3, 3), 1, None),
    "conv4s2_first": Block(_raw_plain("conv4x4s2_first"), None, (0, 4, 4), 1, None),
}


def block_weight(kind, weight, lo=None, hi=None):
    blk = BLOCKS[kind]
    return weight if blk.mode is None else weights.packed(weight, bool(blk.finish[0]), lo, hi, blk.cat)


CONV3_WX = True
CONV3_WX_MIN_WGS = 256


def conv3_wx_applies(n, cin, h, w, cout, *modules) -> bool:
    return (CONV3_WX and not torch.is_grad_enabled() and not any(m.training for m in modules)
            and ops.lib().dvg_tile_policy() == 1 and cin == 64 and w >= 64 and ops.wx_ok(n, cin, h, w, cout)
            and ops.wx_workgroups(n, h, w, cout) >= CONV3_WX_MIN_WGS)


def _skip_half(kind, skip, ps, conv=None):
    if kind == "conv3" and conv is not None and not conv.training and not torch.is_grad_enabled():
        n, c, h, w = skip.shape
        ctot = conv.weight.shape[1]
        if winograd_tile(n, c, h, w, conv.weight.shape[0]) == 4:
            return ops.conv3x3_winograd(skip, weights.winograd(conv.weight, 4, ctot - c, ctot), None, None, act=ACT_NONE)
        if conv3_wx_applies(n, c, h, w, conv.weight.shape[0], conv):
            return ops.conv3x3_wx(skip, weights.wx(conv.weight, ctot - c, ctot), None, None, act=ACT_NONE)
    return BLOCKS[kind].raw(skip, None, ps, None)


_scope = types.SimpleNamespace(passes=1, groups=None, trace=None, share=None)


@contextlib.contextmanager
def _scoped(result=None, **fields):
    prev = {k: getattr(_scope, k) for k in fields}
    vars(_scope).update(fields)
    try:
        yield result
    finally:
        vars(_scope).update(prev)


def bn_passes(k: int):
    return _scoped(passes=int(k))


def bn_momentum(bn, passes=None) -> float:
    m = bn.momentum if bn.momentum is not None else 0.1
    return 1.0 - (1.0 - m) ** (_scope.passes if passes is None else passes)


def bn_passes_now() -> int:
    return _scope.passes


_GROUP_STATS_RECOMPUTE = False


def bn_groups(groups: int, passes=(1, 1, 1)):
    return _scoped(groups=(int(groups),) + tuple(int(k) for k in passes) if groups > 1 else None)


def bn_groups_now() -> int:
    return _scope.groups[0] if _scope.groups else 1


def group_stats(st, u):
    g = bn_groups_now()
    if g == 1:
        return st
    if st is not None and getattr(st, "grouped", 0) == g:
        return st
    ti = getattr(st, "tile_images", 0) if st is not None else 0
    if ti and not _GROUP_STATS_RECOMPUTE and st.shape[0] % g == 0 and (u.shape[0] // g) % ti == 0:
        return st
    u2 = u if u.dim() == 2 else u.permute(0, 2, 3, 1).reshape(-1, u.shape[1])
    return ops.channel_stats(u2, g)


def bn_counter(bn):
    return bn.num_batches_tracked if (bn.track_running_stats and bn.num_batches_tracked is not None) else None


def bn_trace():
    trace = types.SimpleNamespace(entries=[])
    return _scoped(trace, trace=trace.entries)


def replay_bn_trace(entries) -> None:
    for bn, stats, count, passes, groups in entries:
        with _scoped(trace=None, groups=groups, passes=passes):
            _train_bn(bn, stats, count, synced=True)


_SYNC_BN = None


def set_sync_bn(dist=None, group=None) -> None:
    global _SYNC_BN
    if dist is None or not dist.is_initialized() or dist.get_world_size(group) <= 1:
        _SYNC_BN = None
    else:
        _SYNC_BN = (dist, group, dist.get_world_size(group))
    ops.set_sync_bn_state(_SYNC_BN)


def sync_bn_world() -> int:
    return _SYNC_BN[2] if _SYNC_BN is not None else 1


def _train_bn(bn: nn.BatchNorm2d, stats, count, save=False, synced=False):
    grouped, passes = _scope.groups, _scope.passes
    g = grouped[0] if grouped else 1
    if _SYNC_BN is not None and not synced:
        stats = ops.sync_partial_rows(stats, g)
        count = count * _SYNC_BN[2]
    if _scope.trace is not None:
        _scope.trace.append((bn, stats, count, passes, grouped))
    if grouped:
        _, p0, p1, p2 = grouped
        if passes != 1 or count % g:
            raise RuntimeError("grouped BatchNorm: bn_passes must be 1 and the groups must divide the batch")
        momentum, passes, momenta = 0.0, p0 + p2 + (g - 2) * p1, tuple(bn_momentum(bn, k) for k in (p0, p1, p2))
    else:
        momentum, momenta = bn_momentum(bn), None
    return ops.bn_finalize(stats, bn.weight.detach() if bn.weight is not None else None,
                           bn.bias.detach() if bn.bias is not None else None,
                           bn.running_mean if bn.track_running_stats else None,
                           bn.running_var if bn.track_running_stats else None, count // g, bn.eps, momentum, save=save,
                           num_batches_tracked=bn_counter(bn), passes=passes, groups=g, group_momenta=momenta)



SKIP_HOIST = os.environ.get("DVG_SKIP_HOIST", "1") != "0"
UPCONV_AS_CONVT = os.environ.get("DVG_UPCONV_AS_CONVT", "1") != "0"
LAST_PROJ_FUSED = True
_skip_seen = {}


_frozen = {}


def clear_skip_hoist_cache():
    _skip_seen.clear()
    _frozen.clear()


_derived.register("skip_hoist", clear_skip_hoist_cache, _skip_seen.values, skip_keyed=(_skip_seen, _frozen))


def declare_frozen_skips(skips) -> None:
    if not SKIP_HOIST:
        return
    for dead in [k for k, e in _frozen.items() if e[0]() is None]:
        del _frozen[dead]
    for s in skips:
        _frozen[id(s)] = (weakref.ref(s), s._version)


def share_skip_halves():
    return _scoped(share={})


def skip_share_scope():
    return _scope.share


def precompute_skip_half(conv, skip, kind: str) -> None:
    if not SKIP_HOIST or skip is None:
        return
    ctot = conv.weight.shape[BLOCKS[kind].cat]
    s = _skip_half(kind, skip, block_weight(kind, conv.weight, ctot - skip.shape[1], ctot), conv)
    _skip_seen[(id(conv), id(skip))] = [weakref.ref(skip), skip._version, _ver(conv.weight), 1, s]


def _hoisted_skip(conv, x, skip, partial_fn, force=False):
    if skip is None or (not SKIP_HOIST and not force):
        return None
    k = (id(conv), id(skip))
    wkey = _ver(conv.weight)
    ent = _skip_seen.get(k)
    if ent is None or ent[0]() is not skip or ent[1] != skip._version or ent[2] != wkey:
        for dead in [kk for kk, e in _skip_seen.items() if e[0]() is None]:
            del _skip_seen[dead]
        if len(_skip_seen) > 64:
            _skip_seen.clear()
        _skip_seen[k] = ent = [weakref.ref(skip), skip._version, wkey, 1, None]
        fz = _frozen.get(id(skip))
        if not force and (fz is None or fz[0]() is not skip or fz[1] != skip._version):
            return None
    else:
        ent[3] += 1
    px, ps = weights.split_packed(conv.weight, x.shape[1], isinstance(conv, nn.ConvTranspose2d))
    if ent[4] is None:
        ent[4] = partial_fn(ps)
    return px, ent[4]


WINOGRAD_CHAIN = os.environ.get("DVG_WINOGRAD_CHAIN", "1") != "0"


_CHAIN_LEVEL = int(os.environ.get("DVG_WINOGRAD_CHAIN", "3"))


def _chain_to(conv_next, n, c, h, w, pool=False):
    if not (WINOGRAD_CHAIN and WINOGRAD >= 4 and conv_next is not None and not conv_next.training
            and isinstance(conv_next, nn.Conv2d) and conv_next.weight.shape[1] == c and tuple(conv_next.kernel_size) == (3, 3)):
        return False
    if pool:
        return (_CHAIN_LEVEL >= 2 and winograd_tile(n, c, h // 2, w // 2, conv_next.weight.shape[0]) == 4
                and ops.winograd_pool_chain_ok(n, c, h, w))
    if h > 16 and _CHAIN_LEVEL < 2:
        return False
    return winograd_tile(n, c, h, w, conv_next.weight.shape[0]) == 4 and ops.winograd_chain_ok(n, c, h, w)


def _from(res, y_from):
    if not y_from:
        return res
    y, yp = res
    return (y[y_from:] if y_from < y.shape[0] else None), yp


def _hoist_ready(conv, skip) -> bool:
    if not SKIP_HOIST or skip is None:
        return False
    ent = _skip_seen.get((id(conv), id(skip)))
    if ent is not None and ent[0]() is skip and ent[1] == skip._version and ent[2] == _ver(conv.weight):
        return True
    fz = _frozen.get(id(skip))
    return fz is not None and fz[0]() is skip and fz[1] == skip._version


def _chain_up_to(next_up, n, c, h, w, stem=False) -> bool:
    if next_up is None or torch.is_grad_enabled():
        return False
    conv_n, bn_n, skip_n = next_up
    if not (WINOGRAD_CHAIN and _CHAIN_LEVEL >= 3 and WINOGRAD >= 4 and UPCONV_WINOGRAD and isinstance(conv_n, nn.Conv2d)
            and tuple(conv_n.kernel_size) == (3, 3) and not conv_n.training and not bn_n.training and skip_n is not None
            and not isinstance(skip_n, ops.SharedBlocks)):
        return False
    if conv_n.weight.shape[1] - skip_n.shape[1] != c or tuple(skip_n.shape) != (n, skip_n.shape[1], 2 * h, 2 * w):
        return False
    return (2 * h <= _UPCONV_WINO_MAX and winograd_tile(n, c, 2 * h, 2 * w, conv_n.weight.shape[0]) == 4
            and ((h, w) == (4, 4) if stem else ops.winograd_up_chain_ok(n, c, h, w)) and _hoist_ready(conv_n, skip_n))


def _hand_over(next_conv, next_up, n, c, h, w, pool=False):
    if _chain_to(next_conv, n, c, h, w, pool):
        return True
    return "up" if not pool and _chain_up_to(next_up, n, c, h, w) else False


def _bn_act_train(bn, u, st, *, act, slope=0.2, pool=False):
    n, _, h, w = u.shape
    sc, sh = _train_bn(bn, group_stats(st, u), n * h * w)
    return ops.bn_act_apply(u, sc, sh, act=act, slope=slope, pool=pool, inplace=True)


def _train_block(kind, conv, bn, x, skip=None, *, up=False, act, slope, pool=False):
    u, st = BLOCKS[kind].raw(x, skip, block_weight(kind, conv.weight), _bias(conv), up=up, stats=True)
    return _bn_act_train(bn, u, st, act=act, slope=slope, pool=pool)


def _last_proj_applies(next_last, conv, x) -> bool:
    if not LAST_PROJ_FUSED or next_last is None or torch.is_grad_enabled() or not isinstance(next_last, nn.ConvTranspose2d):
        return False
    w = next_last.weight
    return (conv.weight.shape[0] == 64 and w.shape[0] == 64 and tuple(w.shape[2:]) == (3, 3) and 9 * w.shape[1] <= ops.PROJ_MAX_T
            and tuple(next_last.stride) == (1, 1) and tuple(next_last.padding) == (1, 1) and x.shape[2] % 8 == 0
            and x.shape[3] % 8 == 0)


def conv3_bn_act(conv, bn, x, skip=None, *, upsample=False, pool=False, act=ACT_LRELU, slope=0.2, next_conv=None, y_from=0,
                 next_up=None, next_last=None):
    if y_from and (not pool or bn.training or _needs_grad(x, skip, conv.weight, bn.weight)):
        raise RuntimeError("conv3_bn_act: y_from is an eval-mode, no-grad option of the pooled form")
    if isinstance(x, ops.WinoV) and x.up:
        hs = None if (bn.training or not upsample or pool) else \
            _hoisted_skip(conv, x, skip, functools.partial(_skip_half, "conv3", skip, conv=conv), force=True)
        if hs is None:
            raise RuntimeError("conv3_bn_act: an upsampled WinoV needs the eval-mode concat conv with its skip half hoisted")
        sc, sh = folded_affine(conv, bn)
        n, c1, h, w = x.shape
        cout = conv.weight.shape[0]
        return ops.conv3x3_winograd(x, weights.winograd(conv.weight, 4, 0, c1), sc, sh, act=act, slope=slope, upsample=True,
                                    addend=hs[1], to_v=_hand_over(next_conv, None, n, cout, h, w))
    if isinstance(x, ops.WinoV):
        if bn.training or skip is not None or upsample:
            raise RuntimeError("conv3_bn_act: a WinoV input needs an eval-mode plain 3x3 layer")
        sc, sh = folded_affine(conv, bn)
        n, c, h, w = x.shape
        cout = conv.weight.shape[0]
        if winograd_tile(n, c, h, w, cout) != 4:
            raise RuntimeError("conv3_bn_act: WinoV handed to a layer that is not F(4x4,3x3)")
        return ops.conv3x3_winograd(x, weights.winograd(conv.weight, 4), sc, sh, act=act, slope=slope, pool=pool,
                                    to_v=_hand_over(next_conv, next_up, n, cout, h, w, pool), y_from=y_from)
    if _needs_grad(x, skip, conv.weight, bn.weight):
        from .autograd import conv_block_autograd
        return conv_block_autograd("conv3", conv, bn, x, skip, upsample=upsample, pool=pool, act=act, slope=slope)
    _no_shared(skip, "conv3_bn_act")
    if not bn.training:
        sc, sh = folded_affine(conv, bn)
        if not pool:
            hs = _hoisted_skip(conv, x, skip, functools.partial(_skip_half, "conv3", skip, conv=conv))
            if hs is not None:
                if upsample and UPCONV_WINOGRAD:
                    n_, c1_, hx_, wx_ = x.shape
                    cout_ = conv.weight.shape[0]
                    if 2 * hx_ <= _UPCONV_WINO_MAX and winograd_tile(n_, c1_, 2 * hx_, 2 * wx_, cout_) == 4:
                        to_v = not torch.is_grad_enabled() and _hand_over(next_conv, None, n_, cout_, 2 * hx_, 2 * wx_)
                        return ops.conv3x3_winograd(x, weights.winograd(conv.weight, 4, 0, c1_), sc, sh, act=act, slope=slope,
                                                    upsample=True, addend=hs[1], to_v=to_v)
                if upsample and UPCONV_AS_CONVT:
                    if _last_proj_applies(next_last, conv, x):
                        w_last = next_last.weight
                        d = ops.convT4x4s2_proj(x, weights.k4_packed(conv.weight, x.shape[1]), sc, sh,
                                                ops._last_wmat_cached(w_last, 0, 64, 9 * w_last.shape[1]), act=act, slope=slope,
                                                addend=hs[1])
                        return ops.LastProj(d, (x.shape[0], 64, 2 * x.shape[2], 2 * x.shape[3]), w_last)
                    return ops.convT4x4s2(x, None, weights.k4_packed(conv.weight, x.shape[1]), sc, sh, act=act, slope=slope,
                                          addend=hs[1])
                return ops.conv3x3(x, None, hs[0], sc, sh, upsample=upsample, act=act, slope=slope, addend=hs[1])
        if skip is None and not upsample:
            n, c, h, w = x.shape
            cout = conv.weight.shape[0]
            m = winograd_tile(n, c, h, w, cout)
            if m:
                to_v = m == 4 and not torch.is_grad_enabled() and _hand_over(next_conv, next_up, n, cout, h, w, pool)
                return ops.conv3x3_winograd(x, weights.winograd(conv.weight, m), sc, sh, act=act, slope=slope, pool=pool,
                                            to_v=to_v, y_from=y_from)
            if conv3_wx_applies(n, c, h, w, cout, conv, bn):
                return _from(ops.conv3x3_wx(x, weights.wx(conv.weight), sc, sh, act=act, slope=slope, pool=pool), y_from)
        return _from(ops.conv3x3(x, skip, weights.packed(conv.weight), sc, sh, upsample=upsample, act=act, slope=slope,
                                 pool=pool), y_from)
    return _train_block("conv3", conv, bn, x, skip, up=upsample, act=act, slope=slope, pool=pool)


def conv3_first_bn_act(conv, bn, x_nchw, *, act=ACT_LRELU, slope=0.2):
    if _needs_grad(x_nchw, conv.weight, bn.weight):
        from .autograd import conv_block_autograd
        return conv_block_autograd("conv3_first", conv, bn, x_nchw, None, act=act, slope=slope)
    if not bn.training:
        sc, sh = folded_affine(conv, bn)
        return ops.conv3x3_first(x_nchw, conv.weight, sc, sh, act=act, slope=slope)
    return _train_block("conv3_first", conv, bn, x_nchw, act=act, slope=slope)


FIRST_PAIR = True


def first_pair_applies(conv0, bn0, conv1, bn1, x_nchw) -> bool:
    if not FIRST_PAIR or bn0.training or bn1.training or _needs_grad(x_nchw, conv0.weight, bn0.weight, conv1.weight, bn1.weight):
        return False
    n, nc, h, w = x_nchw.shape
    return conv0.out_channels == 64 and conv1.in_channels == 64 and ops.first_pair_ok(n, nc, h, w, conv1.out_channels)


def conv3_first_pair(conv0, bn0, conv1, bn1, x_nchw, *, pool=False, slope=0.2, y_from=0):
    sc0, sh0 = folded_affine(conv0, bn0)
    sc1, sh1 = folded_affine(conv1, bn1)
    n, _, h, w = x_nchw.shape
    if conv3_wx_applies(n, 64, h, w, conv1.out_channels, conv0, bn0, conv1, bn1):
        return ops.conv3x3_first_pair_wx(x_nchw, weights.first_pair_taps(conv0.weight), sc0, sh0, weights.wx(conv1.weight), sc1, sh1,
                                         slope=slope, pool=pool, y_from=y_from)
    return ops.conv3x3_first_pair(x_nchw, weights.first_pair_taps(conv0.weight), sc0, sh0, weights.packed(conv1.weight), sc1, sh1,
                                  slope=slope, pool=pool, y_from=y_from)


def conv4s2_bn_act(conv, bn, x, *, act=ACT_LRELU, slope=0.2):
    if _needs_grad(x, conv.weight, bn.weight):
        from .autograd import conv_block_autograd
        return conv_block_autograd("conv4s2", conv, bn, x, None, act=act, slope=slope)
    if not bn.training:
        sc, sh = folded_affine(conv, bn)
        return ops.conv4x4s2(x, weights.packed(conv.weight), sc, sh, act=act, slope=slope)
    return _train_block("conv4s2", conv, bn, x, act=act, slope=slope)


def conv4s2_first_bn_act(conv, bn, x_nchw, *, act=ACT_LRELU, slope=0.2):
    if _needs_grad(x_nchw, conv.weight, bn.weight):
        from .autograd import conv_block_autograd
        return conv_block_autograd("conv4s2_first", conv, bn, x_nchw, None, act=act, slope=slope)
    if not bn.training:
        sc, sh = folded_affine(conv, bn)
        return ops.conv4x4s2_first(x_nchw, conv.weight, sc, sh, act=act, slope=slope)
    return _train_block("conv4s2_first", conv, bn, x_nchw, act=act, slope=slope)


def convT4s2_bn_act(conv, bn, x, skip=None, *, act=ACT_LRELU, slope=0.2):
    if _needs_grad(x, skip, conv.weight, bn.weight):
        from .autograd import conv_block_autograd
        return conv_block_autograd("convT4s2", conv, bn, x, skip, act=act, slope=slope)
    _no_shared(skip, "convT4s2_bn_act")
    if not bn.training:
        sc, sh = folded_affine(conv, bn)
        hs = _hoisted_skip(conv, x, skip, functools.partial(_skip_half, "convT4s2", skip))
        if hs is not None:
            return ops.convT4x4s2(x, None, hs[0], sc, sh, act=act, slope=slope, addend=hs[1])
        return ops.convT4x4s2(x, skip, weights.packed(conv.weight, True), sc, sh, act=act, slope=slope)
    return _train_block("convT4s2", conv, bn, x, skip, act=act, slope=slope)


def head_bn_tanh(conv, bn, x):
    if _needs_grad(x, conv.weight, bn.weight):
        from .autograd import dense_block_autograd
        return dense_block_autograd("head", conv, bn, x, act=ACT_TANH)
    n, c, h, w = x.shape
    if (h, w) != tuple(conv.kernel_size):
        raise RuntimeError(f"encoder head expects a {conv.kernel_size} map, got {(h, w)}")
    gw = weights.gemm_operand(conv.weight, "head")
    a = x.permute(0, 2, 3, 1).reshape(n, h * w * c)
    k = a.shape[1]
    splitk = max(1, min(64, k // 128))
    if not bn.training:
        sc, sh = folded_affine(conv, bn)
        return ops.gemm_nt(a, gw, sc, sh, act=ACT_TANH, splitk=splitk)
    u = ops.gemm_nt(a, gw, None, _bias(conv), act=ACT_NONE, splitk=splitk)
    u4 = u.view(n, 1, 1, u.shape[1]).permute(0, 3, 1, 2)
    return _bn_act_train(bn, u4, ops.channel_stats(u, bn_groups_now()), act=ACT_TANH).reshape(n, u.shape[1])


def stem_bn_act(conv, bn, vec, *, act=ACT_LRELU, slope=0.2, next_up=None):
    if _needs_grad(vec, conv.weight, bn.weight):
        from .autograd import dense_block_autograd
        return dense_block_autograd("stem", conv, bn, vec, act=act, slope=slope)
    dim, cout, kh, kw = conv.weight.shape
    vec = vec.reshape(-1, dim)
    n = vec.shape[0]
    gw = weights.gemm_operand(conv.weight, "stem")
    if not bn.training:
        sc, sh = folded_affine(conv, bn)
        wt = weights.gemm_operand(conv.weight, "stem_t")
        if wt is not None and (kh, kw) == (4, 4) and cout % 16 == 0 and _chain_up_to(next_up, n, cout, 4, 4, stem=True):
            return ops.stem_up_winograd_input(vec, wt, dim, sc, sh, cout, act=act, slope=slope)
    out = ops.nhwc_empty(n, cout, kh, kw, vec.device)
    out2d = out.permute(0, 2, 3, 1).reshape(n, kh * kw * cout)
    if not bn.training:
        if wt is not None:
            ops.stem_gemm(vec, wt, dim, sc, sh, out2d, period=cout, act=act, slope=slope)
        else:
            ops.gemm_nt(vec, gw, sc, sh, act=act, slope=slope, period=cout, out=out2d)
        return out
    ops.gemm_nt(vec, gw, None, _bias(conv), act=ACT_NONE, period=cout, out=out2d)
    return _bn_act_train(bn, out, ops.channel_stats(out2d.view(n * kh * kw, cout), bn_groups_now()), act=act, slope=slope)


def convT3_last(conv, x, *, act=ACT_SIGMOID):
    if isinstance(x, ops.LastProj):
        return ops.convT_last_two_step(x, None, conv.weight, _bias(conv), conv.weight.shape[1], 3, act=act)
    if _needs_grad(x, conv.weight):
        from .autograd import last_layer_autograd
        return last_layer_autograd("convT3", conv, x, None, act=act)
    return ops.convT_last_two_step(x, None, conv.weight, _bias(conv), conv.weight.shape[1], 3, act=act)


def convT4s2_last(conv, x, skip, *, act=ACT_TANH):
    if _needs_grad(x, skip, conv.weight):
        from .autograd import last_layer_autograd
        return last_layer_autograd("convT4s2", conv, x, skip, act=act)
    _no_shared(skip, "convT4s2_last")
    return ops.convT_last_two_step(x, skip, conv.weight, _bias(conv), conv.weight.shape[1], 4, act=act)
```

dvg_amd/ops/__init__.py:

```python
from ._core import (
    ACT_NONE, ACT_LRELU, ACT_TANH, ACT_SIGMOID, MODE_CONV3, MODE_CONV4S2, MODE_CONVT4S2, _stream, KernelTimer,
    set_timer, _run, _p, _dev_f32, nhwc_empty, is_nhwc, to_nhwc, to_nchw, tile_policy,
)
from .conv import (
    pack_conv_weight, pack_convT_weight, packed_row_floats, pack_igemm_weight, _wp_dims, unpack_conv_weight,
    pack_wx_weight, wx_ok, wx_workgroups, conv3x3_wx,
    unpack_convT_weight, _splitk_ws, _SPLITK_WS, evict_captured_workspaces, _stats_buf, _tile_images, SharedBlocks,
    _MAP_CACHE, shared_map, group_sum, _check_addend, conv3x3, CONV4S2_MAX_FLOATS, conv4x4s2, convT4x4s2,
    PROJ_MAX_T, convT4x4s2_proj,
)
from .winograd import (
    winograd_weight, winograd_ok, WinoV, winograd_chain_ok, winograd_up_chain_ok, winograd_pool_chain_ok,
    conv3x3_winograd, stem_up_winograd_input,
)
from .edge import (
    conv3x3_first, first_pair_ok, conv3x3_first_pair, conv3x3_first_pair_wx, convT3x3_last, conv4x4s2_first, convT4x4s2_last, pixel_proj,
    _SKIP_PROJ_CACHE, clear_skip_proj_cache, _cached_skip_proj, _last_wmat, _last_wmat_cached,
    precompute_skip_proj, LastProj, convT_last_two_step, eval_frames, eval_frames_finn, pairwise_frame_mse, moving_mnist_compose, clip_gather, clip_gather_aug, CLIP_MAX_SHIFT,
    mnist_scale_u8, moving_mnist_compose_u8, frame_mosaic, QUANT_TRUNC, QUANT_NEAREST,
    MOSAIC_BLACK, MOSAIC_RED, MOSAIC_GREEN, MOSAIC_SEL_NONE, MOSAIC_SEL_BEST, MOSAIC_SEL_PICK, MOSAIC_CELL_INTS,
)
from .dense import (
    gemm_nt, lstm_cell, lstm_cell_pre, lstm_cell_bwd, lstm_cell_x, stem_gemm, transpose2d, colsum, GEMM_TN_MAX_ROWS,
    gemm_tn, lstm_gates_bwd, gru_cell, gru_cell_pre, rnn_cell, gru_gates_bwd,
)
from .norm import (
    channel_stats, set_sync_bn_state, sync_bn_state, sync_partial_rows, bn_finalize, bn_act_apply, bn_act_bwd,
)
from .gp import (
    gp_predict, gp_var_norms, gp_trigger_step, gp_trigger_replay, gp_trigger_select, gp_trigger_rows, TRIGGER_NEVER, gp_elbo, gp_elbo_bwd,
    sum_steps, gp_step_group, gp_train_bwd, GP_KERNELS, gp_kernel_code, gp_score, gp_score_slots, gp_score_accumulators,
)
from .backward import (
    _LOSS_W, frame_losses, FRAME_LOSS_KINDS, frame_losses_ext, frame_ssim_loss, mse_sum_grad, conv_wgrad_partial, conv_wgrad_partial_multi, winograd_wgrad_ok,
    winograd_wgrad_partial_multi, wgrad_finish, k4_to_w3, conv_wgrad, wgrad_thin, act_bwd, upsample2x_bwd, adam_step, adam_step_guarded,
    optim_step, ADAM, ADAMW, SGD, RMSPROP, NESTEROV,
)
from .guard import grad_sumsq_blocks, grad_sumsq, grad_guard_finish
from .ema import ema_update_blocks, ema_update
from .lr_schedule import LR_KINDS, lr_schedule_tick
from .validate import val_accumulators, val_accumulate
from .resample import resample_u8, resample_band
from .._lib import check, lib


def __getattr__(name):
    if name == "GP_SCORE_SLOTS":
        from . import gp
        return gp.__getattr__(name)
    raise AttributeError(f"module {__name__!r} has no attribute {name!r}")
```

dvg_amd/ops/_core.py:

```python
from __future__ import annotations

import torch

from .._lib import CONSTANTS, check, lib


ACT_NONE, ACT_LRELU, ACT_TANH, ACT_SIGMOID = (CONSTANTS["ACT_" + k] for k in ("NONE", "LRELU", "TANH", "SIGMOID"))


MODE_CONV3, MODE_CONV4S2, MODE_CONVT4S2 = (CONSTANTS["MODE_" + k] for k in ("CONV3", "CONV4S2", "CONVT4S2"))


def _stream() -> int:
    return torch.cuda.current_stream().cuda_stream


class KernelTimer:

    def __init__(self):
        self.records = []

    def summary(self):
        torch.cuda.synchronize()
        agg = {}
        for name, fl, by, e0, e1, alg in self.records:
            a = agg.setdefault(name, {"launches": 0, "ms": 0.0, "flops": 0.0, "bytes": 0.0, "alg_flops": 0.0})
            a["launches"] += 1
            a["ms"] += e0.elapsed_time(e1)
            a["flops"] += fl
            a["bytes"] += by
            a["alg_flops"] += fl if alg is None else alg
        return agg


_timer = None


def set_timer(t):
    global _timer
    _timer = t


def _run(name, flops, nbytes, fn, *args, alg_flops=None):
    if _timer is None:
        check(fn(*args), name)
        return
    e0, e1 = torch.cuda.Event(enable_timing=True), torch.cuda.Event(enable_timing=True)
    e0.record()
    check(fn(*args), name)
    e1.record()
    _timer.records.append((name, flops, nbytes, e0, e1, alg_flops))


def _p(t):
    return None if t is None else t.data_ptr()


def _dev_f32(t: torch.Tensor, name: str) -> None:
    if not t.is_cuda:
        raise RuntimeError(f"{name}: expected a GPU tensor — the DVG hot path has no CPU fallback")
    if t.dtype != torch.float32:
        raise RuntimeError(f"{name}: expected float32, got {t.dtype}")


def nhwc_empty(n: int, c: int, h: int, w: int, device) -> torch.Tensor:
    return torch.empty((n, h, w, c), device=device, dtype=torch.float32).permute(0, 3, 1, 2)


def is_nhwc(t: torch.Tensor) -> bool:
    if t.dim() != 4:
        return False
    n, c, h, w = t.shape
    return t.stride() == (h * w * c, 1, w * c, c) or (c == 1 and t.is_contiguous()) or \
        (h == 1 and w == 1 and t.is_contiguous())


def to_nhwc(t: torch.Tensor) -> torch.Tensor:
    _dev_f32(t, "to_nhwc")
    if is_nhwc(t):
        return t
    src = t if t.is_contiguous() else t.contiguous()
    n, c, h, w = src.shape
    out = nhwc_empty(n, c, h, w, t.device)
    check(lib().dvg_nchw_to_nhwc(_p(src), _p(out), n, c, h, w, _stream()), "nchw_to_nhwc")
    return out


def to_nchw(t: torch.Tensor) -> torch.Tensor:
    _dev_f32(t, "to_nchw")
    if t.is_contiguous():
        return t
    if not is_nhwc(t):
        return t.contiguous()
    n, c, h, w = t.shape
    out = torch.empty((n, c, h, w), device=t.device, dtype=torch.float32)
    check(lib().dvg_nhwc_to_nchw(_p(t), _p(out), n, c, h, w, _stream()), "nhwc_to_nchw")
    return out


class tile_policy:

    def __init__(self, energy: bool = True):
        self.energy = bool(energy)

    def __enter__(self):
        self.prev = lib().dvg_tile_policy()
        lib().dvg_set_tile_policy(int(self.energy))
        return self

    def __exit__(self, *exc):
        lib().dvg_set_tile_policy(self.prev)
```

dvg_amd/ops/winograd.py:

```python
from __future__ import annotations

import torch

from .._lib import check, lib
from ._core import ACT_LRELU, _dev_f32, _p, _run, _stream, is_nhwc, nhwc_empty
from .conv import packed_row_floats


def winograd_weight(w: torch.Tensor, m: int = 2) -> torch.Tensor:
    _dev_f32(w, "winograd_weight")
    w = w.detach().contiguous()
    co, ci, kh, kw = w.shape
    if (kh, kw) != (3, 3) or ci % 16 or m not in (2, 4):
        raise RuntimeError("winograd_weight: (Cout, Cin % 16 == 0, 3, 3) and m in (2, 4) expected")
    u = torch.empty(((m + 2) ** 2, ci // 16, 1, co, packed_row_floats()), device=w.device, dtype=torch.float32)
    check(lib().dvg_winograd_weight(_p(w), _p(u), co, ci, m, _stream()), "winograd_weight")
    return u


def winograd_ok(n, c, h, w, cout, m: int = 2) -> bool:
    return h % m == 0 and w % m == 0 and c % 64 == 0 and cout % 64 == 0 and (n * (h // m) * (w // m)) % 128 == 0


class WinoV:
    __slots__ = ("v", "shape", "up")

    def __init__(self, v, shape, up=False):
        self.v, self.shape, self.up = v, tuple(shape), bool(up)

    @property
    def device(self):
        return self.v.device

    @property
    def requires_grad(self):
        return False


def winograd_chain_ok(n, c, h, w):
    return h == w and h in (8, 16, 32) and c % 64 == 0 and n > 0


def winograd_up_chain_ok(n, c, h, w):
    return h == w and h == 8 and c % 64 == 0 and n > 0


def winograd_pool_chain_ok(n, c, h, w):
    return h == w and h in (16, 32) and c % 64 == 0 and n > 0


def conv3x3_winograd(x, u, scale, shift, *, act=ACT_LRELU, slope=0.2, pool=False, return_v=False, to_v=False,
                     upsample=False, addend=None, y_from=0):
    from_v = isinstance(x, WinoV)
    if from_v:
        n, c, h, w = x.shape
        if x.up != bool(upsample):
            raise RuntimeError("conv3x3_winograd: a WinoV taken through the upsampling needs upsample=True (and only then)")
    else:
        _dev_f32(x, "conv3x3_winograd.x")
        assert is_nhwc(x), "conv3x3_winograd: x must be NHWC in memory"
        n, c, h, w = x.shape
        if upsample:
            h, w = 2 * h, 2 * w
    cout, npos = u.shape[3], u.shape[0]
    mt = {16: 2, 36: 4}.get(npos, 0)
    if mt == 0 or tuple(u.shape) != (npos, c // 16, 1, cout, packed_row_floats()) or not winograd_ok(n, c, h, w, cout, mt):
        raise RuntimeError(f"conv3x3_winograd: unsupported shape x {tuple(x.shape)} u {tuple(u.shape)}")
    if not 0 <= y_from <= n or (y_from and not pool):
        raise RuntimeError("conv3x3_winograd: y_from needs the pooled output and 0 <= y_from <= N")
    if (from_v or to_v or upsample or addend is not None) and (mt != 4 or return_v):
        raise RuntimeError("conv3x3_winograd: WinoV hand-over / upsample / addend need F(4x4,3x3) and no return_v")
    if addend is not None and pool:
        raise RuntimeError("conv3x3_winograd: addend excludes the pooled output")
    if to_v == "up" and (pool or addend is not None or not winograd_up_chain_ok(n, cout, h, w)):
        raise RuntimeError(f"conv3x3_winograd: to_v='up' unsupported for output {(n, cout, h, w)} pool={pool}")
    if addend is not None:
        _dev_f32(addend, "conv3x3_winograd.addend")
        if tuple(addend.shape) != (n, cout, h, w) or not is_nhwc(addend):
            raise RuntimeError(f"conv3x3_winograd: addend {tuple(addend.shape)} must be NHWC {(n, cout, h, w)}")
    if to_v and to_v != "up" and not (winograd_pool_chain_ok(n, cout, h, w) if pool else winograd_chain_ok(n, cout, h, w)):
        raise RuntimeError(f"conv3x3_winograd: to_v unsupported for output {(n, cout, h, w)} pool={pool}")
    t = n * (h // mt) * (w // mt)
    dev = x.device
    m = torch.empty((npos, t, cout), device=dev, dtype=torch.float32)
    if from_v:
        v = x.v
        if tuple(v.shape) != (npos, t, c):
            raise RuntimeError("conv3x3_winograd: WinoV does not match its shape")
    else:
        v = torch.empty((npos, t, c), device=dev, dtype=torch.float32)
        _run("winograd_input", 0.0, 4.0 * (x.numel() + v.numel()), lib().dvg_winograd_input, _p(x), _p(v), n, h, w, c, mt,
             int(upsample), _stream())
    _run("winograd_gemm", 2.0 * npos * t * c * cout, 4.0 * (v.numel() + m.numel() + u.numel()), lib().dvg_gemm_batched_k16,
         _p(v), _p(u), _p(m), npos, t // 16, 16, c, cout, _stream(), alg_flops=2.0 * n * h * w * cout * 9 * c)
    if to_v and pool:
        y = nhwc_empty(n - y_from, cout, h, w, dev) if y_from < n else None
        vn = torch.empty((npos, t // 4, cout), device=dev, dtype=torch.float32)
        _run("winograd_output_pool_input", 0.0, 4.0 * (m.numel() + (0 if y is None else y.numel()) + vn.numel()),
             lib().dvg_winograd_output_pool_input, _p(m), _p(scale), _p(shift), _p(y), _p(vn), n, h, w, cout, act, slope, y_from,
             _stream())
        return y, WinoV(vn, (n, cout, h // 2, w // 2))
    if to_v == "up":
        vn = torch.empty((npos, 4 * t, cout), device=dev, dtype=torch.float32)
        _run("winograd_output_up_input", 0.0, 4.0 * (m.numel() + vn.numel()), lib().dvg_winograd_output_up_input, _p(m), _p(scale),
             _p(shift), _p(vn), n, h, w, cout, act, slope, _stream())
        return WinoV(vn, (n, cout, 2 * h, 2 * w), up=True)
    if to_v:
        vn = torch.empty((npos, t, cout), device=dev, dtype=torch.float32)
        _run("winograd_output_input", 0.0, 4.0 * (m.numel() + vn.numel()), lib().dvg_winograd_output_input, _p(m), _p(scale),
             _p(shift), _p(vn), n, h, w, cout, act, slope, _p(addend), _stream())
        return WinoV(vn, (n, cout, h, w))
    y = nhwc_empty(n - y_from, cout, h, w, dev) if y_from < n else None
    yp = nhwc_empty(n, cout, h // 2, w // 2, dev) if pool else None
    _run("winograd_output", 0.0, 4.0 * (m.numel() + (0 if y is None else y.numel()) + (0 if yp is None else yp.numel())),
         lib().dvg_winograd_output, _p(m), _p(scale), _p(shift), _p(y), _p(yp), n, h, w, cout, act, slope, mt, _p(addend), y_from,
         _stream())
    if return_v:
        return ((y, yp) if pool else y), v
    return (y, yp) if pool else y


def stem_up_winograd_input(vec, w_kn, k, scale, shift, cout, *, act=ACT_LRELU, slope=0.2):
    _dev_f32(vec, "stem_up_winograd_input.vec")
    if vec.dim() != 2 or vec.stride(1) != 1:
        vec = vec.contiguous().view(vec.shape[0], -1)
    m = vec.shape[0]
    kp, n = w_kn.shape
    if vec.shape[1] != k or n != 16 * cout or cout % 16:
        raise RuntimeError("stem_up_winograd_input: shape mismatch")
    v = torch.empty((36, 4 * m, cout), device=vec.device, dtype=torch.float32)
    _run("stem_up_winograd_input", 2.0 * m * n * k, 4.0 * (m * k + n * k + v.numel()), lib().dvg_stem_up_winograd_input, _p(vec),
         vec.stride(0), _p(w_kn), kp, _p(scale), _p(shift), _p(v), m, cout, k, act, slope, _stream())
    return WinoV(v, (m, cout, 8, 8), up=True)
```

dvg_amd/weights.py:

```python
from __future__ import annotations

import torch

from . import ops
from ._derived import derived


def _span(weight, lo, hi, dim):
    return (None, None, None) if lo is None or (lo == 0 and hi == weight.shape[dim]) else (lo, hi, dim)


def _sliced(weight, lo, hi, dim):
    w = weight.detach()
    if lo is not None:
        w = w[lo:hi] if dim == 0 else w[:, lo:hi]
    return w.contiguous()


def packed(weight, transposed=False, lo=None, hi=None, dim=0):
    lo, hi, dim = _span(weight, lo, hi, dim)
    return derived(weight, ("wp", transposed, lo, hi, dim), (weight,),
                   lambda: ops.pack_igemm_weight(_sliced(weight, lo, hi, dim), transposed))


def wx(weight, lo=None, hi=None):
    lo, hi, dim = _span(weight, lo, hi, 1)
    return derived(weight, ("wx", lo, hi), (weight,), lambda: ops.pack_wx_weight(_sliced(weight, lo, hi, dim)))


def split_packed(weight, c1: int, transposed=False):
    dim = 0 if transposed else 1
    return packed(weight, transposed, 0, c1, dim), packed(weight, transposed, c1, weight.shape[dim], dim)


def winograd(weight, m, lo=None, hi=None, dgrad=False):
    lo, hi, _ = _span(weight, lo, hi, 1)

    def build():
        w = weight.detach()
        if lo is not None:
            w = w[:, lo:hi]
        if dgrad:
            w = w.transpose(0, 1).flip(2, 3)
        return ops.winograd_weight(w.contiguous(), m)

    return derived(weight, ("wino", m, lo, hi, dgrad), (weight,), build)


def k4_weight(weight, c1: int) -> torch.Tensor:
    w = weight.detach()[:, :c1]
    k4 = torch.zeros((w.shape[0], c1, 4, 4), device=w.device, dtype=torch.float32)
    for ty in range(3):
        for tx in range(3):
            k4[:, :, 2 - ty:4 - ty, 2 - tx:4 - tx] += w[:, :, ty:ty + 1, tx:tx + 1]
    return k4.permute(1, 0, 2, 3).contiguous()


def k4_packed(weight, c1: int, adjoint=False):
    def build():
        k4 = derived(weight, ("k4", c1), (weight,), lambda: k4_weight(weight, c1))
        return ops.pack_igemm_weight(k4, transposed=not adjoint)

    return derived(weight, ("k4p", c1, adjoint), (weight,), build)


def transposed(weight):
    return derived(weight, "T", (weight,), lambda: ops.transpose2d(weight.detach()))


def gemm_operand(weight, kind: str):
    def build():
        if kind.endswith("_T"):
            return ops.transpose2d(gemm_operand(weight, kind[:-2]))
        w = weight.detach()
        if kind == "head":
            n, c, kh, kw = w.shape
            return w.permute(0, 2, 3, 1).reshape(n, kh * kw * c).contiguous()
        k, c, kh, kw = w.shape
        if kind == "stem":
            return w.permute(2, 3, 1, 0).reshape(kh * kw * c, k).contiguous()
        gw = None
        if k <= 128 and (kh * kw * c) % 32 == 0:
            gw = torch.zeros((96 if k <= 96 else 128, kh * kw * c), device=w.device, dtype=torch.float32)
            gw[:k] = w.permute(0, 2, 3, 1).reshape(k, kh * kw * c)
        return gw

    if kind not in ("head", "stem", "stem_t", "head_T", "stem_T"):
        raise RuntimeError(kind)
    return derived(weight, ("gw", kind), (weight,), build)


def first_pair_taps(weight):
    return derived(weight, "w_t9x64", (weight,), lambda: weight.detach().reshape(64, 9).t().contiguous())
```

include/dvg_hip.h:

```cpp
#ifndef DVG_HIP_H
#define DVG_HIP_H

#include <stddef.h>
#include <stdint.h>

#ifdef __cplusplus
extern "C" {
#endif

#define DVG_OK 0
#define DVG_ERR_SHAPE 1
#define DVG_ERR_NULL 2
#define DVG_ERR_HIP 3
#define DVG_ERR_ALIGN 4
#define DVG_ACT_NONE 0
#define DVG_ACT_LRELU 1
#define DVG_ACT_TANH 2
#define DVG_ACT_SIGMOID 3
int dvg_abi_version(void);
const char* dvg_last_error(void);
long dvg_stream_capture_id(void* stream);
int dvg_pack_conv_weight(const float* w_oihw, float* w_packed, int cout, int cin, int kh, int kw, void* stream);
int dvg_pack_convT_weight(const float* w_iohw, float* w_packed, int cin, int cout, int kh, int kw, void* stream);
int dvg_unpack_conv_weight(const float* w_packed, float* w_oihw, int cout, int cin, int kh, int kw, void* stream);
int dvg_unpack_convT_weight(const float* w_packed, float* w_iohw, int cin, int cout, int kh, int kw, void* stream);
#define DVG_MODE_CONV3 0
#define DVG_MODE_CONV4S2 1
#define DVG_MODE_CONVT4S2 2
int dvg_conv_first_stats_rows(int ks, int N, int H, int W);
int dvg_mfma_mode(void);
int dvg_packed_row_floats(void);
const char* dvg_build_info(void);
void dvg_set_tile_policy(int energy);
int dvg_tile_policy(void);
int dvg_pack_conv_weight_k16(const float* w, float* w_packed, int cout, int cin, int kh, int kw, int transposed, void* stream);
int dvg_conv_splitk_v2(int mode, int N, int H, int W, int Cin, int Cout);
int dvg_conv_stats_rows_v2(int mode, int N, int H, int W, int Cin, int Cout, int pool, int with_workspace);
int dvg_conv3x3_bn_act_v2(const float* x, const float* skip, const float* w_k16, const float* scale, const float* shift, float* y,
                          float* y_pool, float* stats, int N, int H, int W, int C1, int C2, int Cout, int upsample_x, int act,
                          float slope, float* workspace, long workspace_floats, const float* addend,
                          const int* addend_map, int addend_block, void* stream);
int dvg_conv3x3_first_pair(const float* frame, const float* w0, const float* scale0, const float* shift0, const float* w1_k16,
                           const float* scale1, const float* shift1, float* y, float* y_pool, int N, int H, int W, int Cout, int act, float slope,
                           int y_from , void* stream);
int dvg_pack_conv_weight_wx(const float* w, float* w_packed, int cout, int cin, void* stream);
int dvg_conv3x3_bn_act_wx(const float* x, const float* skip, const float* w_wx, const float* scale, const float* shift, float* y, float* y_pool, int N, int H, int W, int C1, int C2, int Cout, int upsample_x, int act, float slope, const float* addend, const int* addend_map, int addend_block, void* stream);
int dvg_conv3x3_first_pair_wx(const float* frame, const float* w0, const float* scale0, const float* shift0, const float* w1_wx, const float* scale1, const float* shift1, float* y, float* y_pool, int N, int H, int W, int Cout, int act, float slope, int y_from, void* stream);
int dvg_conv4x4s2_bn_act_v2(const float* x, const float* w_k16, const float* scale, const float* shift, float* y, float* stats,
                            int N, int H, int W, int Cin, int Cout, int act, float slope, float* workspace, long workspace_floats, void* stream);
int dvg_convT4x4s2_bn_act_v2(const float* x, const float* skip, const float* w_k16, const float* scale, const float* shift, float* y,
                             float* stats, int N, int H, int W, int C1, int C2, int Cout, int act, float slope, float* workspace,
                             long workspace_floats, const float* addend, const int* addend_map , int addend_block, void* stream);
int dvg_convT4x4s2_bn_act_proj(const float* x, const float* w_k16, const float* scale, const float* shift, const float* proj_w, float* proj_out, int T,
                               int N, int H, int W, int C1, int Cout, int act, float slope, const float* addend, const int* addend_map, int addend_block, void* stream);
int dvg_winograd_weight(const float* w_oihw, float* u_k16, int cout, int cin, int m, void* stream);
int dvg_winograd_input(const float* x, float* v, int N, int H, int W, int C, int m, int upsample, void* stream);
int dvg_gemm_batched_k16(const float* x, const float* w_k16, float* y, int NB, int H, int W, int Cin, int Cout, void* stream);
int dvg_gemm_batched_plan(int NB, int H, int W, int Cin, int Cout, int* tile_w, int* nt, int* ni);
int dvg_winograd_transform_width(long tiles, int C);
int dvg_winograd_output(const float* mm, const float* scale, const float* shift, float* y, float* y_pool, int N, int H,
                        int W, int C, int act, float slope, int m, const float* addend,
                        int y_from , void* stream);
int dvg_winograd_output_input(const float* mm, const float* scale, const float* shift, float* v_next, int N, int H, int W,
                              int C, int act, float slope, const float* addend , void* stream);
int dvg_stem_up_winograd_input(const float* vec, int ldv, const float* w_kn, int KP, const float* scale, const float* shift,
                               float* v_next, int M, int C, int K, int act, float slope, void* stream);
int dvg_winograd_output_up_input(const float* mm, const float* scale, const float* shift, float* v_next, int N, int H, int W,
                                 int C, int act, float slope, void* stream);
int dvg_winograd_output_pool_input(const float* m, const float* scale, const float* shift, float* y, float* v_next, int N,
                                   int H, int W, int C, int act, float slope, int y_from, void* stream);

int dvg_conv3x3_first(const float* x_nchw, const float* w_oihw, const float* scale, const float* shift, float* y, float* stats,
                      int N, int H, int W, int nc, int Cout, int act, float slope, void* stream);

int dvg_convT3x3_last(const float* x, const float* w_iohw, const float* bias, float* y_nchw, int N, int H, int W, int Cin,
                      int nc, int act, void* stream);

int dvg_conv4x4s2_first(const float* x_nchw, const float* w_oihw, const float* scale, const float* shift, float* y, float* stats,
                        int N, int H, int W, int nc, int Cout, int act, float slope, void* stream);

int dvg_convT4x4s2_last(const float* x, const float* skip, const float* w_iohw, const float* bias, float* y_nchw, int N, int H,
                        int W, int C1, int C2, int nc, int act, void* stream);

int dvg_pixel_proj(const float* in, const float* w, float* out, long P, int C, int T, void* stream);

int dvg_convT_gather(const float* d1, const float* d2, const float* bias, float* y_nchw, int ks,
                     int N, int H, int W, int nc, int act,
                     const int* d2_map ,
                     int d2_block, void* stream);


int dvg_channel_stats_rows(long rows);
int dvg_channel_stats(const float* u, float* stats_partial, long rows, int C, int groups, void* stream);
int dvg_channel_stats_pivot(const float* u, float* stats_partial, const float* pivot, long rows, int C, int groups,
                            void* stream);

int dvg_bn_finalize(const float* stats_partial, int nrows, const float* gamma,
                    const float* beta, float* scale, float* shift, float* running_mean,
                    float* running_var, float* save_mean, float* save_invstd,
                    int C, double count, float eps, float momentum,
                    int64_t* num_batches_tracked , int nbt_inc, int groups,
                    float* group_var, void* stream);
int dvg_bn_finalize_pivot(const float* stats_partial, int nrows, const float* pivot, const float* gamma,
                          const float* beta, float* scale, float* shift, float* running_mean, float* running_var,
                          float* save_mean, float* save_invstd, int C, double count, float eps, float momentum,
                          int64_t* num_batches_tracked, int nbt_inc, int groups, float* group_var, void* stream);
int dvg_bn_running_update(const float* mean, const float* unbiased_var, int groups, int C, float mom_first, float mom_mid,
                          float mom_last, float* running_mean, float* running_var, int64_t* num_batches_tracked,
                          int nbt_inc, void* stream);

int dvg_bn_act_apply(const float* u, const float* scale, const float* shift, float* y,
                     float* y_pool, int N, int H, int W, int C, int act, float slope,
                     int group_images, void* stream);

int dvg_gemm_nt_bias_act(const float* a, const float* w, const float* scale, const float* shift, float* out, float* workspace,
                         int M, int N, int K, int lda, int ldo, int period, int splitk, int act, float slope,
                         int accumulate , void* stream);

int dvg_lstm_cell(const float* x, const float* h, const float* c, const float* w_ih, const float* w_hh, const float* b_ih,
                  const float* b_hh, float* h_out, float* c_out, float* gates_out, int B, int H, void* stream);

int dvg_lstm_cell_pre(const float* pre, const float* h, const float* c, const float* w_hh, float* h_out,
                      float* c_out, float* gates_out, int B, int H, void* stream);
int dvg_lstm_cell_bwd(const float* dh_a, const float* dh_b, const float* dc, const float* gates,
                      const float* c_prev, const float* c_new, const float* w_hh_t, float* dG, float* dc_prev,
                      float* dh_prev, int B, int H, void* stream);

int dvg_lstm_cell_x(const float* x, int ldx, int Kx, const float* h, const float* c, const float* w_x, int Kxp,
                    const float* w_hh, const float* bias, float* h_out, float* c_out, int B, int H, void* stream);

int dvg_gru_cell(const float* x, const float* h, const float* w_ih, const float* w_hh, const float* b_ih, const float* b_hh,
                 float* h_out, float* acts_out, int B, int H, void* stream);
int dvg_gru_cell_pre(const float* pre, const float* h, const float* w_hh, const float* b_hn, float* h_out, float* acts_out,
                     int B, int H, void* stream);
int dvg_rnn_cell(const float* x, const float* h, const float* w_ih, const float* w_hh, const float* b_ih, const float* b_hh,
                 float* h_out, int B, int H, void* stream);
int dvg_gru_gates_bwd(const float* dh_a, const float* dh_b, const float* acts, const float* h_prev, float* dGi, float* dGh,
                      float* dh_prev, int B, int H, void* stream);

int dvg_stem_gemm(const float* vec, int ldv, const float* w_kn, int KP, const float* scale, const float* shift,
                  float* out, int ldo, int M, int N, int K, int period, int act, float slope, void* stream);

int dvg_gp_precision(int B, int M, int need_cov);
size_t dvg_gp_lds_bytes(int B, int M, int need_cov);
int dvg_gp_predict(const float* h, const float* z, const float* var_mean, const float* chol_var, const float* mean_const,
                   const float* outputscale, const float* lengthscale, const float* noise, const float* eps, float* mean,
                   float* var, float* sample, float* cov, float* kl, int B, int D, int M, int train_mode, float jitter,
                   int param_period, int step_group, void* stream);
int dvg_gp_step_group(int B, int S, int P, int M);
enum { DVG_GP_KERNEL_RBF = 0, DVG_GP_KERNEL_MATERN12 = 1, DVG_GP_KERNEL_MATERN32 = 2, DVG_GP_KERNEL_MATERN52 = 3 };
int dvg_gp_predict_cov(const float* h, const float* z, const float* var_mean, const float* chol_var, const float* mean_const,
                       const float* outputscale, const float* lengthscale, const float* noise, const float* eps, float* mean,
                       float* var, float* sample, float* cov, float* kl, int B, int D, int M, int train_mode, float jitter,
                       int param_period, int step_group, int cov_kind, void* stream);


int dvg_bn_act_bwd_rows(int N, int H, int W, int pool);
int dvg_bn_act_bwd_reduce(const float* dy, const float* dyp, const float* y, const float* u,
                          float* dp, float* partial, int N, int H, int W, int C, int act,
                          float slope, int groups, void* stream);
int dvg_bn_act_bwd_reduce_centered(const float* dy, const float* dyp, const float* y, const float* u, const float* mean,
                                   float* dp, float* partial, int N, int H, int W, int C, int act, float slope,
                                   int groups, void* stream);
int dvg_bn_bwd_finalize(const float* partial, int nrows, const float* gamma, const float* mean,
                        const float* invstd, float* coefA, float* coefB, float* coefC,
                        float* dgamma, float* dbeta, float* dbias, int C, double count,
                        int train, int accumulate , int groups, void* stream);
int dvg_bn_bwd_finalize_centered(const float* partial, int nrows, const float* gamma, const float* mean,
                                 const float* invstd, float* coefA, float* coefB, float* coefC,
                                 float* dgamma, float* dbeta, float* dbias, int C, double count,
                                 int train, int accumulate, int groups, void* stream);
int dvg_affine3_apply(const float* dp, const float* u, const float* A, const float* B,
                      const float* Cc, float* du, long n, int C, float* sum, int sum_mode,
                      int groups , void* stream);
int dvg_group_sum(const float* src, const int* map, float* dst, int groups, int blocks, long block_elems, void* stream);
int dvg_act_bwd(const float* dy, const float* y, float* dpre, long n, int act, float slope,
                void* stream);
int dvg_upsample2x_bwd(const float* dxu, float* dx, int N, int H, int W, int C, void* stream);
int dvg_colsum(const float* a, float* out, int rows, int C, int accumulate , void* stream);
int dvg_reduce_partials(const float* partial, float* out, int S, long n, void* stream);

int dvg_conv_wgrad_splits(int mode, int N, int H, int W, int Cin, int Cout);
int dvg_conv_wgrad(int mode, const float* x, const float* skip, const float* dout,
                   float* partial, int N, int H, int W, int C1, int C2, int Cout,
                   int upsample_x, void* stream);
int dvg_conv_wgrad_splits_multi(int mode, int N, int H, int W, int Cin, int Cout, int items);
int dvg_conv_wgrad_multi(int mode, int items, const float* const* x, const float* const* skip,
                         const float* const* dout, float* partial, int N, int H, int W, int C1, int C2,
                         int Cout, int upsample_x, void* stream);

int dvg_winograd_wgrad_operands(const float* x, const float* dy, float* v, float* dm, int N, int H, int W, int Cin,
                                int Cout, long t_total, long t_off, void* stream);
int dvg_winograd_wgrad_splits(long t_total, int Cin, int Cout);
int dvg_winograd_wgrad_gemm(const float* dm, const float* v, float* partial, long t_total, int Cin, int Cout, void* stream);
int dvg_winograd_wgrad_gemm_items(const float* dm, const float* const* v_items, int items, long tiles_per_item,
                                  float* partial, int Cin, int Cout, void* stream);
int dvg_winograd_wgrad_reduce(const float* partial, int S, float* packed, int Cin, int Cout, void* stream);

int dvg_wgrad_finish(const float* partial, int S, float* dst, int kind, int kh, int kw, int cout, int cin, int ctot,
                     int c_lo, float beta, void* stream);
int dvg_k4_to_w3(const float* dk4_packed, float* dw, int cout, int c1, int ctot, int c_lo, float beta, void* stream);

int dvg_wgrad_thin_rows(int ks, int N, int Hi, int Wi);
int dvg_wgrad_thin(const float* inp_nchw, const float* dout_nhwc, float* partial, int ks, int N, int Hi, int Wi, int nc, int C, void* stream);

int dvg_moving_mnist_compose(const float* sprites, const int* ids, const int* pos, float* out, int n_sprites, int T, int B, int num_digits, int image_size, int digit_size, void* stream);

int dvg_clip_gather_u8(const uint8_t* pool, const int64_t* first, float* out, int64_t n_frames, int T, int B, int C, int H, int W, int pool_c, void* stream);
int dvg_clip_gather_aug_u8(const uint8_t* pool, const int64_t* first, const int32_t* geom, const float* photo, float* out, int64_t n_frames, int T, int B, int C, int H, int W, int pool_c, void* stream);

int dvg_mnist_scale_u8(const uint8_t* raw, uint8_t* out, int n, int in_size, int out_size, const int* xmin, const int* coef, void* stream);
int dvg_resample_u8_band(const int* ymin_host, int Hin, int Win, int Hout, int Wout, int C, int yk, int* span);
int dvg_resample_u8(const uint8_t* src, uint8_t* dst, int n, int Hin, int Win, int Hout, int Wout, int C, const int* xmin, const int* xcoef, int xk, const int* ymin, const int* ycoef, int yk, const int* ymin_host, void* stream);

int dvg_moving_mnist_compose_u8(const uint8_t* sprites, const int* ids, const int* pos, float* out, int n_sprites, int T, int B, int num_digits, int image_size, int digit_size, void* stream);

int dvg_eval_frames(const float* gt, const float* pred, float* ssim, float* psnr, int n_images, int H, int W,
                    void* stream);

int dvg_eval_frames_finn(const float* gt, const float* pred, float* ssim, float* psnr, float* mse, int n_frames, int C, int H,
                         int W, void* stream);

int dvg_pairwise_frame_mse(const float* samples, float* out, int S, long sample_stride, int frames, long frame_stride, int D,
                           void* stream);

#define DVG_MOSAIC_CELL_INTS 8
#define DVG_MOSAIC_BLACK 0
#define DVG_MOSAIC_RED 1
#define DVG_MOSAIC_GREEN 2
#define DVG_MOSAIC_SEL_NONE 0
#define DVG_MOSAIC_SEL_BEST 1
#define DVG_MOSAIC_SEL_PICK 2
#define DVG_QUANT_TRUNC 0
#define DVG_QUANT_NEAREST 1
int dvg_frame_mosaic(const float* src0, long n0, const float* src1, long n1, const float* src2, long n2, int nc, int H,
                     int W, const int* cells, int F, int R, int Cc, int cell_h, int cell_w, int pad_y, int pad_x, int oy,
                     int ox, const long* best, int n_best, const int* picks, int n_pick_rows, int pick_k,
                     const unsigned char* labels, int n_labels, int lh, int lw, int quant, unsigned char* out,
                     void* stream);

int dvg_adam_step(float* param, const float* grad, float* exp_avg, float* exp_avg_sq, long n, float lr, float beta1,
                  float beta2, float eps, float weight_decay, int step, const int* step_dev, void* stream);

int dvg_gemm_tn(const float* a, const float* b, float* out, float* colsum0, float* colsum1, int R, int M, int N,
                int lda, int ldb, int ldo, int accumulate, int colsum_accumulate, void* stream);
int dvg_lstm_gates_bwd(const float* dh, const float* dc, const float* gates, const float* c_prev, const float* c_new, float* dG,
                       float* dc_prev, int B, int H, void* stream);

int dvg_gp_bwd_precision(int B, int M);
size_t dvg_gp_bwd_lds_bytes(int B, int M);
int dvg_gp_bwd_chunk(int B, int M);
int dvg_gp_train_bwd(const float* h, const float* z, const float* var_mean, const float* chol_var, const float* mean_const,
                     const float* outputscale, const float* lengthscale, const float* gmean, const float* gvar, const float* gkl,
                     float* dh, float* dz, float* dm, float* dls, float* dc, float* ds, float* dell, int B, int D, int M,
                     float jitter, int param_period, int step_group, void* stream);
int dvg_gp_train_bwd_cov(const float* h, const float* z, const float* var_mean, const float* chol_var, const float* mean_const,
                         const float* outputscale, const float* lengthscale, const float* gmean, const float* gvar,
                         const float* gkl, float* dh, float* dz, float* dm, float* dls, float* dc, float* ds, float* dell, int B,
                         int D, int M, float jitter, int param_period, int step_group, int cov_kind, void* stream);
int dvg_sum_steps_multi(const float* const* src, float* const* dst, const long* n, int count, int S, void* stream);

int dvg_gp_elbo(const float* mean, const float* var, const float* kl, const float* target, long t_stride_d,
                long t_stride_b, const float* raw_noise, float* elbo, int B, int D, int num_data,
                int noise_period , void* stream);
int dvg_gp_elbo_bwd(const float* mean, const float* var, const float* kl, const float* target, long t_stride_d, long t_stride_b,
                    const float* raw_noise, const float* gelbo, float* gmean, float* gvar, float* gkl, float* gtarget,
                    float* graw_noise, int B, int D, int num_data, int noise_period, void* stream);

int dvg_nchw_to_nhwc(const float* x, float* y, int N, int C, int H, int W, void* stream);
int dvg_nhwc_to_nchw(const float* x, float* y, int N, int C, int H, int W, void* stream);
void dvg_debug_set_clockbuf(void* buf, unsigned records);
void dvg_debug_set_gp_clockbuf(void* buf, unsigned records);
void dvg_debug_set_wgrad_clockbuf(void* buf, unsigned records);

int dvg_gp_var_norms(const float* var, float* norms, int D, int B, void* stream);
int dvg_gp_trigger_step(const float* var, int D, int B, int col, float* ctx, int window, float coef, int* flag, float* values, float* thresholds, int* flags, int slot, void* stream);
int dvg_gp_trigger_replay(const float* values, int n, const float* ctx0, int window, float coef, int* flags, float* thresholds, void* stream);
int dvg_gp_trigger_select(const int* flag, const float* sample_db, const float* h_pred, float* vec, int D, int B, int n_state, long state_elems, const float* const* state_old, const float* const* state_new, float* const* state_out, void* stream);
int dvg_gp_trigger_rows(const float* var, const float* sample_db, const float* h_pred, float* vec, int D, int B, float* win, int window, int pos, int decide, float coef, int step, int min_gap, int* last, float* values, float* thresholds, int* flags, int slot, void* stream);
int dvg_frame_losses_blocks(long elems);
int dvg_frame_losses(const float* pred, const float* target, float* sums, float* dpred, long n, int S, int K, const float* w,
                     float* partial, void* stream);
int dvg_mse_sum_grad(const float* a, const float* b, float* sum, float* da, long n, float scale, void* stream);
int dvg_frame_losses_ext_blocks(int S, long planes, int H, int W);
int dvg_frame_losses_ext(const float* pred, const float* target, float* sums, float* dpred, int S, int K, long planes, int H, int W,
                         int kind, float eps, const float* w_pix, const float* w_gdl, float* partial, void* stream);
int dvg_frame_ssim_loss_blocks(int S, long planes, int H, int W);
int dvg_frame_ssim_loss(const float* pred, const float* target, float* sums, float* dpred, int S, int K, long planes, int H, int W,
                        const float* w_ssim, int accumulate, double* partial, void* stream);
int dvg_zero_tick(float* g, long n, int* t0, int* t1, int* t2, int* t3, void* stream);
int dvg_grad_sumsq_blocks(long n);
int dvg_grad_sumsq(const float* g, long n, double* partials, void* stream);
int dvg_grad_guard_finish(const double* partials, int nblocks, double max_norm, int skip, float* stat, int* counters, void* stream);
int dvg_adam_step_guarded(float* param, const float* grad, float* exp_avg, float* exp_avg_sq, long n, float lr, float beta1, float beta2,
                          float eps, float weight_decay, int step, const int* step_dev, const float* stat, int* skips_dev, void* stream);
int dvg_lr_schedule_tick(int kind, int W, int N, int K, double R, double G, int* iter_dev, float* scale_dev, void* stream);
int dvg_adam_step_scheduled(float* param, const float* grad, float* exp_avg, float* exp_avg_sq, long n, float lr, float beta1,
                            float beta2, float eps, float weight_decay, int step, const int* step_dev, const float* stat,
                            int* skips_dev, const float* lr_scale_dev, void* stream);
int dvg_optim_step(int rule, float* param, const float* grad, float* m, float* v, long n, float lr, float a, float b, float eps, float weight_decay, int flags,
                   const uint8_t* decay_mask, int step, const int* step_dev, const float* stat, int* skips_dev, const float* lr_scale_dev, void* stream);
int dvg_ema_update_blocks(long n);
int dvg_ema_update(float* ema, const float* param, long n, double decay, const int* updates_dev, double* partials, void* stream);
int dvg_val_accumulate(const float* ssim, const float* psnr, const float* mse, int B, int S, int T, double* acc, long long* cnt,
                       int* best, void* stream);
int dvg_gp_score_slots(int* acc_slots, int* cnt_slots);
int dvg_gp_score(const float* mean, const float* var, const float* noise, int noise_period, const float* target, long t_stride_r, long t_stride_b, int B, int R, double* acc, long long* cnt, void* stream);

#ifdef __cplusplus
}
#endif
#endif
```

Measured before the change: 53500 frames/s.

## Skip dead Winograd F(4x4,3x3) positions for nearest-upsampled inputs

For 2x nearest-upsampled inputs, the Winograd input transform has a row and column (index 2) that are always zero. The change stores only the 25 live positions instead of 36, for the input transforms, the stem-up transform and the output kernels. The batched GEMM then runs over 25 positions, with its tile chosen as if there were 36. This cuts GEMM work and transform traffic by about a third on the upsampled decoder layers, at the cost of extra template variants and a separate set of precomputed weights.

```diff
diff --git a/dvg_amd/csrc/conv_igemm2.hip b/dvg_amd/csrc/conv_igemm2.hip
--- a/dvg_amd/csrc/conv_igemm2.hip
+++ b/dvg_amd/csrc/conv_igemm2.hip
@@ -1599,8 +1599,8 @@
     return launch2<M2_CONVT4S2, 1, 8, 8, 1, false, true>(p, H, W, nullptr, 0, (hipStream_t)stream);
 }
 
-extern "C" int dvg_gemm_batched_k16(const float* x, const float* w_k16, float* y, int NB, int H, int W, int Cin, int Cout,
-                                    void* stream) {
+static int gemm_batched(const float* x, const float* w_k16, float* y, int NB, int nb_tile, int H, int W, int Cin, int Cout,
+                        void* stream) {
     Igemm2Params p{x, nullptr, w_k16, nullptr, nullptr, y, nullptr, nullptr, NB, H, W, Cin, 0, Cout, 0, DVG_ACT_NONE, 0.f,
                    0, 0, 0, 0, 0, 1, 0, nullptr};
     if (int e = checks2(p, "dvg_gemm_batched_k16")) return e;
@@ -1612,7 +1612,7 @@
     const long workspace_floats = 0;
     const int Hg = H, Wg = W, ti = 1, th = 8;
     int tw, nt;
-    DVG_REQUIRE(gemm_tile(NB, Hg, Wg, Cout, &tw, &nt) == 0, DVG_ERR_SHAPE, "dvg_gemm_batched_k16: no tile for %dx%d", H, W);
+    DVG_REQUIRE(gemm_tile(nb_tile, Hg, Wg, Cout, &tw, &nt) == 0, DVG_ERR_SHAPE, "dvg_gemm_batched_k16: no tile for %dx%d", H, W);
 #if DVG_BF16X3
     if (nt == 2) return launch2<M2_GEMM, 1, 8, 16, 2>(p, Hg, Wg, workspace, workspace_floats, (hipStream_t)stream);
 #endif
@@ -1621,10 +1621,29 @@
     return fail(DVG_ERR_SHAPE, "dvg_gemm_batched_k16: no kernel");
 }
 
-extern "C" int dvg_gemm_batched_plan(int NB, int H, int W, int Cin, int Cout, int* tile_w, int* nt, int* ni) {
-    if (!tile_w || !nt || !ni || NB <= 0 || H <= 0 || W <= 0 || Cin <= 0 || Cout <= 0) return -1;
+extern "C" int dvg_gemm_batched_k16(const float* x, const float* w_k16, float* y, int NB, int H, int W, int Cin, int Cout,
+                                    void* stream) {
+    return gemm_batched(x, w_k16, y, NB, NB, H, W, Cin, Cout, stream);
+}
+
+extern "C" int dvg_gemm_batched_k16_as(const float* x, const float* w_k16, float* y, int NB, int NB_as, int H, int W, int Cin,
+                                       int Cout, void* stream) {
+    DVG_REQUIRE(NB > 0 && NB_as >= NB, DVG_ERR_SHAPE, "dvg_gemm_batched_k16_as: NB=%d, NB_as=%d (NB_as >= NB > 0 needed)", NB, NB_as);
+    return gemm_batched(x, w_k16, y, NB, NB_as, H, W, Cin, Cout, stream);
+}
+
+static int gemm_plan(int NB, int nb_tile, int H, int W, int Cin, int Cout, int* tile_w, int* nt, int* ni) {
+    if (!tile_w || !nt || !ni || NB <= 0 || nb_tile < NB || H <= 0 || W <= 0 || Cin <= 0 || Cout <= 0) return -1;
     if (Cin % (16 * DVG_GEMM_GT) || Cout % 64 || H % 8 || W % 8) return -1;
-    if (gemm_tile(NB, H, W, Cout, tile_w, nt)) return -1;
+    if (gemm_tile(nb_tile, H, W, Cout, tile_w, nt)) return -1;
     *ni = gemm_images_per_wg(*tile_w, *nt, NB, H, W, Cout);
     return 0;
 }
+
+extern "C" int dvg_gemm_batched_plan(int NB, int H, int W, int Cin, int Cout, int* tile_w, int* nt, int* ni) {
+    return gemm_plan(NB, NB, H, W, Cin, Cout, tile_w, nt, ni);
+}
+
+extern "C" int dvg_gemm_batched_plan_as(int NB, int NB_as, int H, int W, int Cin, int Cout, int* tile_w, int* nt, int* ni) {
+    return gemm_plan(NB, NB_as, H, W, Cin, Cout, tile_w, nt, ni);
+}
diff --git a/dvg_amd/csrc/winograd.hip b/dvg_amd/csrc/winograd.hip
--- a/dvg_amd/csrc/winograd.hip
+++ b/dvg_amd/csrc/winograd.hip
@@ -162,6 +162,11 @@
     o[3] = b + 8.f * d + q[5];
 }
 
+__device__ __forceinline__ constexpr bool wino_dead(int a, int b) { return a == 2 || b == 2; }
+__device__ __forceinline__ constexpr int wino_pos(bool live, int a, int b) {
+    return live ? (a - (a > 2)) * 5 + (b - (b > 2)) : a * 6 + b;
+}
+
 __global__ void winograd4_weight_kernel(const float* __restrict__ w, float* __restrict__ u, int cout, int cin) {
     const float G[6][3] = {{0.25f, 0.f, 0.f}, {-1.f / 6, -1.f / 6, -1.f / 6}, {-1.f / 6, 1.f / 6, -1.f / 6},
                            {1.f / 24, 1.f / 12, 1.f / 6}, {1.f / 24, -1.f / 12, 1.f / 6}, {0.f, 0.f, 1.f}};
@@ -191,7 +196,7 @@
     wrow_drain();
 }
 
-template <typename V>
+template <typename V, bool LIVE = false>
 __global__ __launch_bounds__(256) void winograd4_input_kernel(const float* __restrict__ x, float* __restrict__ v, int N,
                                                               int H, int W, int C4, long Tt, long t_off, int up) {
     const int Ht = H >> 2, Wt = W >> 2, Hs = H >> up, Ws = W >> up;
@@ -220,10 +225,12 @@
         }
 #pragma unroll
         for (int a = 0; a < 6; ++a) {
+            if (LIVE && a == 2) continue;
             V o[6];
             bt4(e[a], o);
 #pragma unroll
-            for (int b = 0; b < 6; ++b) reinterpret_cast<V*>(v)[((size_t)(a * 6 + b) * Tt + t_off + t) * C4 + c4] = o[b];
+            for (int b = 0; b < 6; ++b)
+                if (!(LIVE && b == 2)) reinterpret_cast<V*>(v)[((size_t)wino_pos(LIVE, a, b) * Tt + t_off + t) * C4 + c4] = o[b];
         }
     }
 }
@@ -272,8 +279,7 @@
     }
 }
 
-template <bool POOL, typename V>
-
+template <bool POOL, typename V, bool MLIVE = false>
 __global__ __launch_bounds__(256) void winograd4_output_kernel(const float* __restrict__ m, const float* __restrict__ scale,
                                                                const float* __restrict__ shift, float* __restrict__ y,
                                                                float* __restrict__ y_pool, int N, int H, int W, int C4,
@@ -293,7 +299,9 @@
         for (int b = 0; b < 6; ++b) {
             V q[6];
 #pragma unroll
-            for (int a = 0; a < 6; ++a) q[a] = reinterpret_cast<const V*>(m)[((size_t)(a * 6 + b) * T + t) * C4 + c4];
+            for (int a = 0; a < 6; ++a)
+                q[a] = (MLIVE && wino_dead(a, b)) ? vzero<V>()
+                                                  : reinterpret_cast<const V*>(m)[((size_t)wino_pos(MLIVE, a, b) * T + t) * C4 + c4];
             V col[4];
             at4(q, col);
 #pragma unroll
@@ -337,7 +345,7 @@
     }
 }
 
-template <int HW>
+template <int HW, bool MLIVE = false>
 __global__ __launch_bounds__(256) void winograd4_out_in_kernel(const float* __restrict__ m, const float* __restrict__ scale,
                                                                const float* __restrict__ shift, float* __restrict__ v, int N,
                                                                int C, int act, float slope, const float* __restrict__ addend) {
@@ -353,7 +361,8 @@
         for (int b = 0; b < 6; ++b) {
             float q[6];
 #pragma unroll
-            for (int a = 0; a < 6; ++a) q[a] = m[((size_t)(a * 6 + b) * T + t) * C + c];
+            for (int a = 0; a < 6; ++a)
+                q[a] = (MLIVE && wino_dead(a, b)) ? 0.f : m[((size_t)wino_pos(MLIVE, a, b) * T + t) * C + c];
             float col[4];
             at4(q, col);
 #pragma unroll
@@ -396,7 +405,7 @@
     }
 }
 
-template <int HW, int CS, typename V, bool POOL, int NT, bool UP = false>
+template <int HW, int CS, typename V, bool POOL, int NT, bool UP = false, bool MLIVE = false, bool VLIVE = false>
 __global__ __launch_bounds__(NT) void winograd4_chain_kernel(const float* __restrict__ m, const float* __restrict__ scale,
                                                              const float* __restrict__ shift, float* __restrict__ y,
                                                              float* __restrict__ v, int N, int C, int act, float slope,
@@ -404,6 +413,7 @@
     constexpr int VN = VecN<V>::N;
     constexpr int WT = HW / 4, TI = WT * WT;
     static_assert(!(POOL && UP), "pool and upsample exclude each other");
+    static_assert(!VLIVE || UP, "only the input transform of an upsampled map has dead positions");
     constexpr int SS = POOL ? HW / 2 : HW;
     constexpr int S2 = UP ? 2 * HW : SS;
     constexpr int WT2 = S2 / 4, TI2 = WT2 * WT2;
@@ -423,7 +433,9 @@
         for (int b = 0; b < 6; ++b) {
             V q[6];
 #pragma unroll
-            for (int a = 0; a < 6; ++a) q[a] = __builtin_nontemporal_load(reinterpret_cast<const V*>(m) + ((size_t)(a * 6 + b) * T + t) * CVg + cg);
+            for (int a = 0; a < 6; ++a)
+                q[a] = (MLIVE && wino_dead(a, b)) ? vzero<V>()
+                                                  : __builtin_nontemporal_load(reinterpret_cast<const V*>(m) + ((size_t)wino_pos(MLIVE, a, b) * T + t) * CVg + cg);
             V col[4];
             at4(q, col);
 #pragma unroll
@@ -493,20 +505,22 @@
         }
 #pragma unroll
         for (int a = 0; a < 6; ++a) {
+            if (VLIVE && a == 2) continue;
             V o[6];
             bt4(e[a], o);
 #pragma unroll
-            for (int b = 0; b < 6; ++b) reinterpret_cast<V*>(v)[((size_t)(a * 6 + b) * T2 + t2) * CVg + cg] = o[b];
-        }
-    }
-}
-
-template <int HW, int CS, typename V, bool POOL, int NT, bool UP = false>
+            for (int b = 0; b < 6; ++b)
+                if (!(VLIVE && b == 2)) reinterpret_cast<V*>(v)[((size_t)wino_pos(VLIVE, a, b) * T2 + t2) * CVg + cg] = o[b];
+        }
+    }
+}
+
+template <int HW, int CS, typename V, bool POOL, int NT, bool UP = false, bool MLIVE = false, bool VLIVE = false>
 static int launch_chain(const float* mm, const float* scale, const float* shift, float* y, float* v, int N, int C, int act,
                         float slope, hipStream_t st, const float* addend = nullptr, int y_from = 0) {
     constexpr int S2 = POOL ? HW / 2 : HW;
     constexpr size_t lds = (size_t)S2 * S2 * CS * 4;
-    auto kern = winograd4_chain_kernel<HW, CS, V, POOL, NT, UP>;
+    auto kern = winograd4_chain_kernel<HW, CS, V, POOL, NT, UP, MLIVE, VLIVE>;
     static bool attr = false;
     if (!attr && lds > 48 * 1024) {
         hipError_t e = hipFuncSetAttribute(reinterpret_cast<const void*>(kern), hipFuncAttributeMaxDynamicSharedMemorySize, (int)lds);
@@ -518,7 +532,7 @@
     return check_launch("winograd4_chain");
 }
 
-template <int KP>
+template <int KP, bool LIVE = false>
 __global__ __launch_bounds__(256) void stem_up_input_kernel(const float* __restrict__ vec, int ldv, const float* __restrict__ wt,
                                                             const float* __restrict__ scale, const float* __restrict__ shift,
                                                             float* __restrict__ v, int M, int C, int K, int act, float slope) {
@@ -578,10 +592,12 @@
         float* dst = v + t * C + blockIdx.x * 16 + ucl;
 #pragma unroll
         for (int a = 0; a < 6; ++a) {
+            if (LIVE && a == 2) continue;
             float o[6];
             bt4(e[a], o);
 #pragma unroll
-            for (int b = 0; b < 6; ++b) dst[(size_t)(a * 6 + b) * T * C] = o[b];
+            for (int b = 0; b < 6; ++b)
+                if (!(LIVE && b == 2)) dst[(size_t)wino_pos(LIVE, a, b) * T * C] = o[b];
         }
     }
 }
@@ -638,6 +654,23 @@
             hipLaunchKernelGGL(winograd4_input_kernel<float>, dim3(wgrid(tiles * C)), dim3(256), 0, st, x, v, N, H, W, C, tiles, 0L, up);
     }
     return check_launch("dvg_winograd_input");
+}
+
+extern "C" int dvg_winograd_input_up_live(const float* x, float* v, int N, int H, int W, int C, void* stream) {
+    DVG_REQUIRE(x && v, DVG_ERR_NULL, "dvg_winograd_input_up_live: NULL pointer");
+    DVG_REQUIRE(N > 0 && H > 0 && W > 0 && H % 4 == 0 && W % 4 == 0 && C > 0 && C % 4 == 0, DVG_ERR_SHAPE,
+                "dvg_winograd_input_up_live: H and W multiples of 4, C %% 4 == 0 needed");
+    DVG_REQUIRE(aligned16(x) && aligned16(v), DVG_ERR_ALIGN, "dvg_winograd_input_up_live: alignment");
+    const long tiles = (long)N * (H / 4) * (W / 4);
+    const hipStream_t st = (hipStream_t)stream;
+    const int cw = wino4_width(tiles, C);
+    if (cw == 4)
+        hipLaunchKernelGGL((winograd4_input_kernel<f32x4, true>), dim3(wgrid(tiles * (C / 4))), dim3(256), 0, st, x, v, N, H, W, C / 4, tiles, 0L, 1);
+    else if (cw == 2)
+        hipLaunchKernelGGL((winograd4_input_kernel<f32x2, true>), dim3(wgrid(tiles * (C / 2))), dim3(256), 0, st, x, v, N, H, W, C / 2, tiles, 0L, 1);
+    else
+        hipLaunchKernelGGL((winograd4_input_kernel<float, true>), dim3(wgrid(tiles * C)), dim3(256), 0, st, x, v, N, H, W, C, tiles, 0L, 1);
+    return check_launch("dvg_winograd_input_up_live");
 }
 
 extern "C" int dvg_winograd_transform_width(long tiles, int C) {
@@ -707,9 +740,30 @@
     return check_launch("dvg_winograd_output_input");
 }
 
-extern "C" int dvg_stem_up_winograd_input(const float* vec, int ldv, const float* w_kn, int KP, const float* scale,
-                                          const float* shift, float* v_next, int M, int C, int K, int act, float slope,
-                                          void* stream) {
+extern "C" int dvg_winograd_output_input_live(const float* mm, const float* scale, const float* shift, float* v_next, int N,
+                                              int H, int W, int C, int act, float slope, const float* addend, void* stream) {
+    DVG_REQUIRE(mm && v_next, DVG_ERR_NULL, "dvg_winograd_output_input_live: NULL pointer");
+    DVG_REQUIRE(aligned16(addend), DVG_ERR_ALIGN, "dvg_winograd_output_input_live: addend alignment");
+    DVG_REQUIRE(N > 0 && H == W && (H == 8 || H == 16 || H == 32) && C > 0 && C % 64 == 0, DVG_ERR_SHAPE,
+                "dvg_winograd_output_input_live: 8x8, 16x16 or 32x32 maps, C %% 64 == 0 needed (got %dx%d, C=%d)", H, W, C);
+    DVG_REQUIRE(act >= 0 && act <= 3, DVG_ERR_SHAPE, "dvg_winograd_output_input_live: bad act");
+    DVG_REQUIRE(aligned16(mm) && aligned16(v_next), DVG_ERR_ALIGN, "dvg_winograd_output_input_live: alignment");
+    const hipStream_t st = (hipStream_t)stream;
+    if (H == 8) {
+        hipLaunchKernelGGL((winograd4_out_in_kernel<8, true>), dim3((unsigned)((long)N * (C / 64))), dim3(256), 0, st, mm, scale,
+                           shift, v_next, N, C, act, slope, addend);
+        return check_launch("dvg_winograd_output_input_live");
+    }
+    if (H == 32)
+        return launch_chain<32, 32, f32x4, false, 512, false, true>(mm, scale, shift, nullptr, v_next, N, C, act, slope, st, addend);
+    if ((long)N * (C / 64) < 1024)
+        return launch_chain<16, 32, float, false, 512, false, true>(mm, scale, shift, nullptr, v_next, N, C, act, slope, st, addend);
+    return launch_chain<16, 64, f32x2, false, 512, false, true>(mm, scale, shift, nullptr, v_next, N, C, act, slope, st, addend);
+}
+
+template <bool LIVE>
+static int stem_up_input(const float* vec, int ldv, const float* w_kn, int KP, const float* scale, const float* shift,
+                         float* v_next, int M, int C, int K, int act, float slope, void* stream) {
     DVG_REQUIRE(vec && w_kn && v_next, DVG_ERR_NULL, "dvg_stem_up_winograd_input: NULL pointer");
     DVG_REQUIRE(M > 0 && C > 0 && C % 16 == 0 && K > 0 && K <= KP && (KP == 96 || KP == 128) && ldv >= K, DVG_ERR_SHAPE,
                 "dvg_stem_up_winograd_input: bad shape M=%d C=%d K=%d KP=%d (C %% 16 == 0, KP 96 or 128)", M, C, K, KP);
@@ -717,23 +771,49 @@
     DVG_REQUIRE(aligned16(v_next), DVG_ERR_ALIGN, "dvg_stem_up_winograd_input: alignment");
     const dim3 grid(C / 16, (M + 7) / 8);
     if (KP == 96)
-        hipLaunchKernelGGL(stem_up_input_kernel<96>, grid, dim3(256), 0, (hipStream_t)stream, vec, ldv, w_kn, scale, shift, v_next,
-                           M, C, K, act, slope);
+        hipLaunchKernelGGL((stem_up_input_kernel<96, LIVE>), grid, dim3(256), 0, (hipStream_t)stream, vec, ldv, w_kn, scale, shift,
+                           v_next, M, C, K, act, slope);
     else
-        hipLaunchKernelGGL(stem_up_input_kernel<128>, grid, dim3(256), 0, (hipStream_t)stream, vec, ldv, w_kn, scale, shift, v_next,
-                           M, C, K, act, slope);
+        hipLaunchKernelGGL((stem_up_input_kernel<128, LIVE>), grid, dim3(256), 0, (hipStream_t)stream, vec, ldv, w_kn, scale, shift,
+                           v_next, M, C, K, act, slope);
     return check_launch("dvg_stem_up_winograd_input");
+}
+
+extern "C" int dvg_stem_up_winograd_input(const float* vec, int ldv, const float* w_kn, int KP, const float* scale,
+                                          const float* shift, float* v_next, int M, int C, int K, int act, float slope,
+                                          void* stream) {
+    return stem_up_input<false>(vec, ldv, w_kn, KP, scale, shift, v_next, M, C, K, act, slope, stream);
+}
+
+extern "C" int dvg_stem_up_winograd_input_live(const float* vec, int ldv, const float* w_kn, int KP, const float* scale,
+                                               const float* shift, float* v_next, int M, int C, int K, int act, float slope,
+                                               void* stream) {
+    return stem_up_input<true>(vec, ldv, w_kn, KP, scale, shift, v_next, M, C, K, act, slope, stream);
 }
 
 extern "C" int dvg_winograd_output_up_input(const float* mm, const float* scale, const float* shift, float* v_next, int N, int H,
                                             int W, int C, int act, float slope, void* stream) {
     DVG_REQUIRE(mm && v_next, DVG_ERR_NULL, "dvg_winograd_output_up_input: NULL pointer");
-    DVG_REQUIRE(N > 0 && H == W && H == 8 && C > 0 && C % 64 == 0, DVG_ERR_SHAPE,
-                "dvg_winograd_output_up_input: 8x8 maps, C %% 64 == 0 needed (got %dx%d, C=%d)", H, W, C);
+    DVG_REQUIRE(N > 0 && H == W && (H == 8 || H == 16) && C > 0 && C % 64 == 0, DVG_ERR_SHAPE,
+                "dvg_winograd_output_up_input: 8x8 or 16x16 maps, C %% 64 == 0 needed (got %dx%d, C=%d)", H, W, C);
     DVG_REQUIRE(act >= 0 && act <= 3, DVG_ERR_SHAPE, "dvg_winograd_output_up_input: bad act");
     DVG_REQUIRE(aligned16(mm) && aligned16(v_next), DVG_ERR_ALIGN, "dvg_winograd_output_up_input: alignment");
     const hipStream_t st = (hipStream_t)stream;
+    if (H == 16) return launch_chain<16, 32, float, false, 512, true>(mm, scale, shift, nullptr, v_next, N, C, act, slope, st);
     return launch_chain<8, 32, float, false, 512, true>(mm, scale, shift, nullptr, v_next, N, C, act, slope, st);
+}
+
+extern "C" int dvg_winograd_output_up_input_live(const float* mm, const float* scale, const float* shift, float* v_next, int N,
+                                                 int H, int W, int C, int act, float slope, void* stream) {
+    DVG_REQUIRE(mm && v_next, DVG_ERR_NULL, "dvg_winograd_output_up_input_live: NULL pointer");
+    DVG_REQUIRE(N > 0 && H == W && (H == 8 || H == 16) && C > 0 && C % 64 == 0, DVG_ERR_SHAPE,
+                "dvg_winograd_output_up_input_live: 8x8 or 16x16 maps, C %% 64 == 0 needed (got %dx%d, C=%d)", H, W, C);
+    DVG_REQUIRE(act >= 0 && act <= 3, DVG_ERR_SHAPE, "dvg_winograd_output_up_input_live: bad act");
+    DVG_REQUIRE(aligned16(mm) && aligned16(v_next), DVG_ERR_ALIGN, "dvg_winograd_output_up_input_live: alignment");
+    const hipStream_t st = (hipStream_t)stream;
+    if (H == 16)
+        return launch_chain<16, 32, float, false, 512, true, false, true>(mm, scale, shift, nullptr, v_next, N, C, act, slope, st);
+    return launch_chain<8, 32, float, false, 512, true, false, true>(mm, scale, shift, nullptr, v_next, N, C, act, slope, st);
 }
 
 extern "C" int dvg_winograd_output_pool_input(const float* mm, const float* scale, const float* shift, float* y, float* v_next,
@@ -783,3 +863,24 @@
     }
     return check_launch("dvg_winograd_output");
 }
+
+extern "C" int dvg_winograd_output_live(const float* m, const float* scale, const float* shift, float* y, int N, int H, int W,
+                                        int C, int act, float slope, const float* addend, void* stream) {
+    DVG_REQUIRE(m && y, DVG_ERR_NULL, "dvg_winograd_output_live: NULL pointer");
+    DVG_REQUIRE(N > 0 && H > 0 && W > 0 && H % 4 == 0 && W % 4 == 0 && C > 0 && C % 4 == 0, DVG_ERR_SHAPE,
+                "dvg_winograd_output_live: H and W multiples of 4, C %% 4 == 0 needed");
+    DVG_REQUIRE(act >= 0 && act <= 3, DVG_ERR_SHAPE, "dvg_winograd_output_live: bad act");
+    DVG_REQUIRE(aligned16(m) && aligned16(y) && aligned16(scale) && aligned16(shift) && aligned16(addend), DVG_ERR_ALIGN,
+                "dvg_winograd_output_live: alignment");
+    const hipStream_t st = (hipStream_t)stream;
+    const long tiles = (long)N * (H / 4) * (W / 4);
+#define W4OUT(V_, CW_)                                                                                                         \
+    hipLaunchKernelGGL((winograd4_output_kernel<false, V_, true>), dim3(wgrid(tiles * (C / CW_))), dim3(256), 0, st, m, scale, \
+                       shift, y, (float*)nullptr, N, H, W, C / CW_, act, slope, addend, 0)
+    const int cw = wino4_width(tiles, C);
+    if (cw == 4) W4OUT(f32x4, 4);
+    else if (cw == 2) W4OUT(f32x2, 2);
+    else W4OUT(float, 1);
+#undef W4OUT
+    return check_launch("dvg_winograd_output_live");
+}
diff --git a/dvg_amd/fused.py b/dvg_amd/fused.py
--- a/dvg_amd/fused.py
+++ b/dvg_amd/fused.py
@@ -42,6 +42,7 @@
 
 UPCONV_WINOGRAD = True
 _UPCONV_WINO_MAX = 16
+UPCONV_WINO_LIVE = True
 
 
 def folded_affine(conv: nn.Module, bn: nn.BatchNorm2d):
@@ -400,8 +401,9 @@
         sc, sh = folded_affine(conv, bn)
         n, c1, h, w = x.shape
         cout = conv.weight.shape[0]
-        return ops.conv3x3_winograd(x, weights.winograd(conv.weight, 4, 0, c1), sc, sh, act=act, slope=slope, upsample=True,
-                                    addend=hs[1], to_v=_hand_over(next_conv, None, n, cout, h, w))
+        u = weights.winograd_live(conv.weight, 0, c1) if x.live else weights.winograd(conv.weight, 4, 0, c1)
+        return ops.conv3x3_winograd(x, u, sc, sh, act=act, slope=slope, upsample=True, addend=hs[1],
+                                    to_v=_hand_over(next_conv, None, n, cout, h, w), live=x.live)
     if isinstance(x, ops.WinoV):
         if bn.training or skip is not None or upsample:
             raise RuntimeError("conv3_bn_act: a WinoV input needs an eval-mode plain 3x3 layer")
@@ -410,8 +412,9 @@
         cout = conv.weight.shape[0]
         if winograd_tile(n, c, h, w, cout) != 4:
             raise RuntimeError("conv3_bn_act: WinoV handed to a layer that is not F(4x4,3x3)")
-        return ops.conv3x3_winograd(x, weights.winograd(conv.weight, 4), sc, sh, act=act, slope=slope, pool=pool,
-                                    to_v=_hand_over(next_conv, next_up, n, cout, h, w, pool), y_from=y_from)
+        to_v = _hand_over(next_conv, next_up, n, cout, h, w, pool)
+        return ops.conv3x3_winograd(x, weights.winograd(conv.weight, 4), sc, sh, act=act, slope=slope, pool=pool, to_v=to_v,
+                                    y_from=y_from, up_live=UPCONV_WINO_LIVE and to_v == "up")
     if _needs_grad(x, skip, conv.weight, bn.weight):
         from .autograd import conv_block_autograd
         return conv_block_autograd("conv3", conv, bn, x, skip, upsample=upsample, pool=pool, act=act, slope=slope)
@@ -426,8 +429,10 @@
                     cout_ = conv.weight.shape[0]
                     if 2 * hx_ <= _UPCONV_WINO_MAX and winograd_tile(n_, c1_, 2 * hx_, 2 * wx_, cout_) == 4:
                         to_v = not torch.is_grad_enabled() and _hand_over(next_conv, None, n_, cout_, 2 * hx_, 2 * wx_)
-                        return ops.conv3x3_winograd(x, weights.winograd(conv.weight, 4, 0, c1_), sc, sh, act=act, slope=slope,
-                                                    upsample=True, addend=hs[1], to_v=to_v)
+                        live = UPCONV_WINO_LIVE and not torch.is_grad_enabled()
+                        u = weights.winograd_live(conv.weight, 0, c1_) if live else weights.winograd(conv.weight, 4, 0, c1_)
+                        return ops.conv3x3_winograd(x, u, sc, sh, act=act, slope=slope, upsample=True, addend=hs[1], to_v=to_v,
+                                                    live=live)
                 if upsample and UPCONV_AS_CONVT:
                     if _last_proj_applies(next_last, conv, x):
                         w_last = next_last.weight
@@ -445,7 +450,7 @@
             if m:
                 to_v = m == 4 and not torch.is_grad_enabled() and _hand_over(next_conv, next_up, n, cout, h, w, pool)
                 return ops.conv3x3_winograd(x, weights.winograd(conv.weight, m), sc, sh, act=act, slope=slope, pool=pool,
-                                            to_v=to_v, y_from=y_from)
+                                            to_v=to_v, y_from=y_from, up_live=UPCONV_WINO_LIVE and to_v == "up")
             if conv3_wx_applies(n, c, h, w, cout, conv, bn):
                 return _from(ops.conv3x3_wx(x, weights.wx(conv.weight), sc, sh, act=act, slope=slope, pool=pool), y_from)
         return _from(ops.conv3x3(x, skip, weights.packed(conv.weight), sc, sh, upsample=upsample, act=act, slope=slope,
@@ -549,7 +554,7 @@
         sc, sh = folded_affine(conv, bn)
         wt = weights.gemm_operand(conv.weight, "stem_t")
         if wt is not None and (kh, kw) == (4, 4) and cout % 16 == 0 and _chain_up_to(next_up, n, cout, 4, 4, stem=True):
-            return ops.stem_up_winograd_input(vec, wt, dim, sc, sh, cout, act=act, slope=slope)
+            return ops.stem_up_winograd_input(vec, wt, dim, sc, sh, cout, act=act, slope=slope, live=UPCONV_WINO_LIVE)
     out = ops.nhwc_empty(n, cout, kh, kw, vec.device)
     out2d = out.permute(0, 2, 3, 1).reshape(n, kh * kw * cout)
     if not bn.training:
diff --git a/dvg_amd/ops/__init__.py b/dvg_amd/ops/__init__.py
--- a/dvg_amd/ops/__init__.py
+++ b/dvg_amd/ops/__init__.py
@@ -10,7 +10,7 @@
     PROJ_MAX_T, convT4x4s2_proj,
 )
 from .winograd import (
-    winograd_weight, winograd_ok, WinoV, winograd_chain_ok, winograd_up_chain_ok, winograd_pool_chain_ok,
+    winograd_weight, winograd_ok, WinoV, LIVE_POSITIONS, winograd_chain_ok, winograd_up_chain_ok, winograd_pool_chain_ok,
     conv3x3_winograd, stem_up_winograd_input,
 )
 from .edge import (
diff --git a/dvg_amd/ops/_core.py b/dvg_amd/ops/_core.py
--- a/dvg_amd/ops/_core.py
+++ b/dvg_amd/ops/_core.py
@@ -1,4 +1,6 @@
 from __future__ import annotations
+
+import collections
 
 import torch
 
@@ -23,7 +25,7 @@
     def summary(self):
         torch.cuda.synchronize()
         agg = {}
-        for name, fl, by, e0, e1, alg in self.records:
+        for name, fl, by, e0, e1, alg, _ in self.records:
             a = agg.setdefault(name, {"launches": 0, "ms": 0.0, "flops": 0.0, "bytes": 0.0, "alg_flops": 0.0})
             a["launches"] += 1
             a["ms"] += e0.elapsed_time(e1)
@@ -31,6 +33,9 @@
             a["bytes"] += by
             a["alg_flops"] += fl if alg is None else alg
         return agg
+
+    def entry_points(self):
+        return collections.Counter(r[6] for r in self.records)
 
 
 _timer = None
@@ -49,7 +54,7 @@
     e0.record()
     check(fn(*args), name)
     e1.record()
-    _timer.records.append((name, flops, nbytes, e0, e1, alg_flops))
+    _timer.records.append((name, flops, nbytes, e0, e1, alg_flops, getattr(fn, "__name__", "")))
 
 
 def _p(t):
diff --git a/dvg_amd/ops/winograd.py b/dvg_amd/ops/winograd.py
--- a/dvg_amd/ops/winograd.py
+++ b/dvg_amd/ops/winograd.py
@@ -22,11 +22,16 @@
     return h % m == 0 and w % m == 0 and c % 64 == 0 and cout % 64 == 0 and (n * (h // m) * (w // m)) % 128 == 0
 
 
+LIVE_POSITIONS = tuple(a * 6 + b for a in range(6) if a != 2 for b in range(6) if b != 2)
+
+
 class WinoV:
-    __slots__ = ("v", "shape", "up")
+    __slots__ = ("v", "shape", "up", "live")
 
-    def __init__(self, v, shape, up=False):
-        self.v, self.shape, self.up = v, tuple(shape), bool(up)
+    def __init__(self, v, shape, up=False, live=False):
+        self.v, self.shape, self.up, self.live = v, tuple(shape), bool(up), bool(live)
+        if self.live and not self.up:
+            raise RuntimeError("WinoV: only the transform of an upsampled map has a live-only form")
 
     @property
     def device(self):
@@ -42,7 +47,7 @@
 
 
 def winograd_up_chain_ok(n, c, h, w):
-    return h == w and h == 8 and c % 64 == 0 and n > 0
+    return h == w and h in (8, 16) and c % 64 == 0 and n > 0
 
 
 def winograd_pool_chain_ok(n, c, h, w):
@@ -50,7 +55,7 @@
 
 
 def conv3x3_winograd(x, u, scale, shift, *, act=ACT_LRELU, slope=0.2, pool=False, return_v=False, to_v=False,
-                     upsample=False, addend=None, y_from=0):
+                     upsample=False, addend=None, y_from=0, live=False, up_live=False):
     from_v = isinstance(x, WinoV)
     if from_v:
         n, c, h, w = x.shape
@@ -63,7 +68,15 @@
         if upsample:
             h, w = 2 * h, 2 * w
     cout, npos = u.shape[3], u.shape[0]
-    mt = {16: 2, 36: 4}.get(npos, 0)
+    if live and (not upsample or pool):
+        raise RuntimeError("conv3x3_winograd: live needs upsample=True and no pooled output")
+    if (npos == 25) != bool(live) or (from_v and x.live != bool(live)):
+        raise RuntimeError("conv3x3_winograd: live needs the 25 live slabs of U and a live WinoV (and only then)")
+    if up_live and to_v != "up":
+        raise RuntimeError("conv3x3_winograd: up_live needs to_v='up'")
+    if live and to_v == "up":
+        raise RuntimeError("conv3x3_winograd: a live layer does not hand over through another upsampling")
+    mt = {16: 2, 36: 4, 25: 4}.get(npos, 0)
     if mt == 0 or tuple(u.shape) != (npos, c // 16, 1, cout, packed_row_floats()) or not winograd_ok(n, c, h, w, cout, mt):
         raise RuntimeError(f"conv3x3_winograd: unsupported shape x {tuple(x.shape)} u {tuple(u.shape)}")
     if not 0 <= y_from <= n or (y_from and not pool):
@@ -89,10 +102,18 @@
             raise RuntimeError("conv3x3_winograd: WinoV does not match its shape")
     else:
         v = torch.empty((npos, t, c), device=dev, dtype=torch.float32)
-        _run("winograd_input", 0.0, 4.0 * (x.numel() + v.numel()), lib().dvg_winograd_input, _p(x), _p(v), n, h, w, c, mt,
-             int(upsample), _stream())
-    _run("winograd_gemm", 2.0 * npos * t * c * cout, 4.0 * (v.numel() + m.numel() + u.numel()), lib().dvg_gemm_batched_k16,
-         _p(v), _p(u), _p(m), npos, t // 16, 16, c, cout, _stream(), alg_flops=2.0 * n * h * w * cout * 9 * c)
+        if live:
+            _run("winograd_input", 0.0, 4.0 * (x.numel() + v.numel()), lib().dvg_winograd_input_up_live, _p(x), _p(v), n, h, w,
+                 c, _stream())
+        else:
+            _run("winograd_input", 0.0, 4.0 * (x.numel() + v.numel()), lib().dvg_winograd_input, _p(x), _p(v), n, h, w, c, mt,
+                 int(upsample), _stream())
+    if live:
+        _run("winograd_gemm", 2.0 * npos * t * c * cout, 4.0 * (v.numel() + m.numel() + u.numel()), lib().dvg_gemm_batched_k16_as,
+             _p(v), _p(u), _p(m), npos, 36, t // 16, 16, c, cout, _stream(), alg_flops=2.0 * n * h * w * cout * 9 * c)
+    else:
+        _run("winograd_gemm", 2.0 * npos * t * c * cout, 4.0 * (v.numel() + m.numel() + u.numel()), lib().dvg_gemm_batched_k16,
+             _p(v), _p(u), _p(m), npos, t // 16, 16, c, cout, _stream(), alg_flops=2.0 * n * h * w * cout * 9 * c)
     if to_v and pool:
         y = nhwc_empty(n - y_from, cout, h, w, dev) if y_from < n else None
         vn = torch.empty((npos, t // 4, cout), device=dev, dtype=torch.float32)
@@ -101,15 +122,22 @@
              _stream())
         return y, WinoV(vn, (n, cout, h // 2, w // 2))
     if to_v == "up":
-        vn = torch.empty((npos, 4 * t, cout), device=dev, dtype=torch.float32)
-        _run("winograd_output_up_input", 0.0, 4.0 * (m.numel() + vn.numel()), lib().dvg_winograd_output_up_input, _p(m), _p(scale),
+        vn = torch.empty((25 if up_live else 36, 4 * t, cout), device=dev, dtype=torch.float32)
+        _run("winograd_output_up_input", 0.0, 4.0 * (m.numel() + vn.numel()),
+             lib().dvg_winograd_output_up_input_live if up_live else lib().dvg_winograd_output_up_input, _p(m), _p(scale),
              _p(shift), _p(vn), n, h, w, cout, act, slope, _stream())
-        return WinoV(vn, (n, cout, 2 * h, 2 * w), up=True)
+        return WinoV(vn, (n, cout, 2 * h, 2 * w), up=True, live=up_live)
     if to_v:
-        vn = torch.empty((npos, t, cout), device=dev, dtype=torch.float32)
-        _run("winograd_output_input", 0.0, 4.0 * (m.numel() + vn.numel()), lib().dvg_winograd_output_input, _p(m), _p(scale),
+        vn = torch.empty((36, t, cout), device=dev, dtype=torch.float32)
+        _run("winograd_output_input", 0.0, 4.0 * (m.numel() + vn.numel()),
+             lib().dvg_winograd_output_input_live if live else lib().dvg_winograd_output_input, _p(m), _p(scale),
              _p(shift), _p(vn), n, h, w, cout, act, slope, _p(addend), _stream())
         return WinoV(vn, (n, cout, h, w))
+    if live:
+        y = nhwc_empty(n, cout, h, w, dev)
+        _run("winograd_output", 0.0, 4.0 * (m.numel() + y.numel()), lib().dvg_winograd_output_live, _p(m), _p(scale),
+             _p(shift), _p(y), n, h, w, cout, act, slope, _p(addend), _stream())
+        return y
     y = nhwc_empty(n - y_from, cout, h, w, dev) if y_from < n else None
     yp = nhwc_empty(n, cout, h // 2, w // 2, dev) if pool else None
     _run("winograd_output", 0.0, 4.0 * (m.numel() + (0 if y is None else y.numel()) + (0 if yp is None else yp.numel())),
@@ -120,7 +148,7 @@
     return (y, yp) if pool else y
 
 
-def stem_up_winograd_input(vec, w_kn, k, scale, shift, cout, *, act=ACT_LRELU, slope=0.2):
+def stem_up_winograd_input(vec, w_kn, k, scale, shift, cout, *, act=ACT_LRELU, slope=0.2, live=False):
     _dev_f32(vec, "stem_up_winograd_input.vec")
     if vec.dim() != 2 or vec.stride(1) != 1:
         vec = vec.contiguous().view(vec.shape[0], -1)
@@ -128,7 +156,8 @@
     kp, n = w_kn.shape
     if vec.shape[1] != k or n != 16 * cout or cout % 16:
         raise RuntimeError("stem_up_winograd_input: shape mismatch")
-    v = torch.empty((36, 4 * m, cout), device=vec.device, dtype=torch.float32)
-    _run("stem_up_winograd_input", 2.0 * m * n * k, 4.0 * (m * k + n * k + v.numel()), lib().dvg_stem_up_winograd_input, _p(vec),
+    v = torch.empty((25 if live else 36, 4 * m, cout), device=vec.device, dtype=torch.float32)
+    _run("stem_up_winograd_input", 2.0 * m * n * k, 4.0 * (m * k + n * k + v.numel()),
+         lib().dvg_stem_up_winograd_input_live if live else lib().dvg_stem_up_winograd_input, _p(vec),
          vec.stride(0), _p(w_kn), kp, _p(scale), _p(shift), _p(v), m, cout, k, act, slope, _stream())
-    return WinoV(v, (m, cout, 8, 8), up=True)
+    return WinoV(v, (m, cout, 8, 8), up=True, live=live)
diff --git a/dvg_amd/weights.py b/dvg_amd/weights.py
--- a/dvg_amd/weights.py
+++ b/dvg_amd/weights.py
@@ -47,6 +47,16 @@
     return derived(weight, ("wino", m, lo, hi, dgrad), (weight,), build)
 
 
+def winograd_live(weight, lo=None, hi=None):
+    lo, hi, _ = _span(weight, lo, hi, 1)
+
+    def build():
+        u = winograd(weight, 4, lo, hi)
+        return u.index_select(0, torch.tensor(ops.LIVE_POSITIONS, device=u.device))
+
+    return derived(weight, ("wino_live", lo, hi), (weight,), build)
+
+
 def k4_weight(weight, c1: int) -> torch.Tensor:
     w = weight.detach()[:, :c1]
     k4 = torch.zeros((w.shape[0], c1, 4, 4), device=w.device, dtype=torch.float32)
diff --git a/include/dvg_hip.h b/include/dvg_hip.h
--- a/include/dvg_hip.h
+++ b/include/dvg_hip.h
@@ -58,17 +58,18 @@
 int dvg_gemm_batched_k16(const float* x, const float* w_k16, float* y, int NB, int H, int W, int Cin, int Cout, void* stream);
 int dvg_gemm_batched_plan(int NB, int H, int W, int Cin, int Cout, int* tile_w, int* nt, int* ni);
 int dvg_winograd_transform_width(long tiles, int C);
-int dvg_winograd_output(const float* mm, const float* scale, const float* shift, float* y, float* y_pool, int N, int H,
-                        int W, int C, int act, float slope, int m, const float* addend,
-                        int y_from , void* stream);
-int dvg_winograd_output_input(const float* mm, const float* scale, const float* shift, float* v_next, int N, int H, int W,
-                              int C, int act, float slope, const float* addend , void* stream);
-int dvg_stem_up_winograd_input(const float* vec, int ldv, const float* w_kn, int KP, const float* scale, const float* shift,
-                               float* v_next, int M, int C, int K, int act, float slope, void* stream);
-int dvg_winograd_output_up_input(const float* mm, const float* scale, const float* shift, float* v_next, int N, int H, int W,
-                                 int C, int act, float slope, void* stream);
-int dvg_winograd_output_pool_input(const float* m, const float* scale, const float* shift, float* y, float* v_next, int N,
-                                   int H, int W, int C, int act, float slope, int y_from, void* stream);
+int dvg_winograd_output(const float* mm, const float* scale, const float* shift, float* y, float* y_pool, int N, int H, int W, int C, int act, float slope, int m, const float* addend, int y_from , void* stream);
+int dvg_winograd_output_input(const float* mm, const float* scale, const float* shift, float* v_next, int N, int H, int W, int C, int act, float slope, const float* addend , void* stream);
+int dvg_stem_up_winograd_input(const float* vec, int ldv, const float* w_kn, int KP, const float* scale, const float* shift, float* v_next, int M, int C, int K, int act, float slope, void* stream);
+int dvg_winograd_output_up_input(const float* mm, const float* scale, const float* shift, float* v_next, int N, int H, int W, int C, int act, float slope, void* stream);
+int dvg_winograd_output_pool_input(const float* m, const float* scale, const float* shift, float* y, float* v_next, int N, int H, int W, int C, int act, float slope, int y_from, void* stream);
+int dvg_winograd_input_up_live(const float* x, float* v, int N, int H, int W, int C, void* stream);
+int dvg_stem_up_winograd_input_live(const float* vec, int ldv, const float* w_kn, int KP, const float* scale, const float* shift, float* v_next, int M, int C, int K, int act, float slope, void* stream);
+int dvg_winograd_output_up_input_live(const float* mm, const float* scale, const float* shift, float* v_next, int N, int H, int W, int C, int act, float slope, void* stream);
+int dvg_gemm_batched_k16_as(const float* x, const float* w_k16, float* y, int NB, int NB_as, int H, int W, int Cin, int Cout, void* stream);
+int dvg_gemm_batched_plan_as(int NB, int NB_as, int H, int W, int Cin, int Cout, int* tile_w, int* nt, int* ni);
+int dvg_winograd_output_input_live(const float* mm, const float* scale, const float* shift, float* v_next, int N, int H, int W, int C, int act, float slope, const float* addend, void* stream);
+int dvg_winograd_output_live(const float* mm, const float* scale, const float* shift, float* y, int N, int H, int W, int C, int act, float slope, const float* addend, void* stream);
 
 int dvg_conv3x3_first(const float* x_nchw, const float* w_oihw, const float* scale, const float* shift, float* y, float* stats,
                       int N, int H, int W, int nc, int Cout, int act, float slope, void* stream);
```

New measurement: 54370 frames/s, median of 6. 1.02x the previous value.
